# gssales/gaussian-splatting-reflection

Hardware: AMD Instinct MI355X
Metric: train_step_views_per_s (fwd+bwd, 1e6 Gaussians @1080p, surfel rasterizer + reflection path) (higher is better)
Workload: dtype f32

## Files before the change

### gaussian-splatting-reflection_amd/csrc/gsr_common.hip

```cpp
#include "gsr_internal.hpp"
#include <cstdarg>
#include <string>
#include <initializer_list>
#include <vector>
#include <mutex>
#include "gsr_sort.hpp"
#include <rocprim/device/device_scan.hpp>
#include <rocprim/iterator/counting_iterator.hpp>
#include <rocprim/iterator/transform_iterator.hpp>

namespace gsr {

static thread_local char g_err[512] = "";
void set_error(const char* fmt, ...) {
	va_list ap;
	va_start(ap, fmt);
	vsnprintf(g_err, sizeof(g_err), fmt, ap);
	va_end(ap);
}


struct ProfRec {
	int stage;
	hipEvent_t e0, e1;
};
static bool g_prof_on = false;
static std::vector<ProfRec*> g_prof_recs;
static std::vector<ProfRec*> g_prof_free;
static std::mutex g_prof_mu;

StageTimer::StageTimer(int stage_, hipStream_t stream_) : stage(stage_), stream(stream_), rec(nullptr) {
	if (!g_prof_on) return;
	std::lock_guard<std::mutex> lk(g_prof_mu);
	ProfRec* r = nullptr;
	if (!g_prof_free.empty()) {
		r = g_prof_free.back();
		g_prof_free.pop_back();
	} else {
		r = new ProfRec();
		if (hipEventCreate(&r->e0) != hipSuccess || hipEventCreate(&r->e1) != hipSuccess) { delete r; return; }
	}
	r->stage = stage;
	(void)hipEventRecord(r->e0, stream);
	rec = r;
}
StageTimer::~StageTimer() {
	if (!rec) return;
	ProfRec* r = (ProfRec*)rec;
	(void)hipEventRecord(r->e1, stream);
	std::lock_guard<std::mutex> lk(g_prof_mu);
	g_prof_recs.push_back(r);
}

static int g_opt_cull = 1;
int option_cull() { return g_opt_cull; }
static int g_opt_dev = 0;
int option_dev() { return g_opt_dev; }
unsigned long long* dev_pair_counter() {
	static std::mutex mu;
	static unsigned long long* words[64];
	int dev = 0;
	if (hipGetDevice(&dev) != hipSuccess || dev < 0 || dev >= 64) return nullptr;
	std::lock_guard<std::mutex> lk(mu);
	if (!words[dev]) {
		if (hipMalloc((void**)&words[dev], sizeof(unsigned long long)) != hipSuccess) { (void)hipGetLastError(); words[dev] = nullptr; return nullptr; }
		if (hipMemset(words[dev], 0, sizeof(unsigned long long)) != hipSuccess) return nullptr;
	}
	return words[dev];
}
static int g_opt_emit_items = 0;
static int g_opt_mailbox = 1;
static int option_mailbox() { return g_opt_mailbox; }
static int g_opt_sort_driver = GSR_ONESWEEP_DRIVER;
int option_sort_driver() { return GSR_ONESWEEP_DRIVER && g_opt_sort_driver; }

uint32_t higher_msb(uint32_t n) {
	uint32_t msb = sizeof(n) * 4;
	uint32_t step = msb;
	while (step > 1) {
		step /= 2;
		if (n >> msb) msb += step;
		else msb -= step;
	}
	if (n >> msb) msb++;
	return msb;
}

using SortConfig = rocprim::radix_sort_config<rocprim::default_config, rocprim::default_config, rocprim::default_config, 65536>;
#ifndef DEPTH_SORT_BS
#define DEPTH_SORT_BS 1024
#endif
#ifndef DEPTH_SORT_IPT
#define DEPTH_SORT_IPT 4
#endif
#define DEPTH_SORT_SHAPE DEPTH_SORT_BS, DEPTH_SORT_IPT, 8
#define DEPTH_KEY_BITS 31u
#define DEPTH_KEY_PLACES 4u
#ifndef TILE_SORT_IPT
#define TILE_SORT_IPT 16
#endif
#ifndef TILE_SORT_BITS
#define TILE_SORT_BITS 8
#endif
#ifndef TILE_SORT_BS
#define TILE_SORT_BS 1024
#endif
#define TILE_SORT_SHAPE TILE_SORT_BS, TILE_SORT_IPT, TILE_SORT_BITS
#ifndef TILE_SORT_SMALL_FROM
#define TILE_SORT_SMALL_FROM 9000000
#endif
#define TILE_SORT_SHAPE_SMALL TILE_SORT_BS, (TILE_SORT_IPT / 2), TILE_SORT_BITS
#define TILE_SORT_SHAPE_SMALL7 TILE_SORT_BS, (TILE_SORT_IPT / 2), 7
static bool tile_sort_small(size_t R) { return R >= (size_t)TILE_SORT_SMALL_FROM; }
static bool tile_sort_7bit(size_t R, int end_bit) { return tile_sort_small(R) && end_bit > 7 && end_bit <= 14; }
template <class F>
static auto with_tile_sort(size_t R, int end_bit, F&& f) {
	if (tile_sort_7bit(R, end_bit)) return f(RadixSort<TILE_SORT_SHAPE_SMALL7, SortConfig>{});
	if (tile_sort_small(R)) return f(RadixSort<TILE_SORT_SHAPE_SMALL, SortConfig>{});
	return f(RadixSort<TILE_SORT_SHAPE, SortConfig>{});
}
using DepthSort = RadixSort<DEPTH_SORT_SHAPE, SortConfig>;

struct OrderRect {
	const uint32_t* rect;
	int packed;
	__host__ __device__ unsigned long long operator()(uint32_t i) const {
		uint32_t hi = 0u;
		if (packed) {
			const uint2 r = reinterpret_cast<const uint2*>(rect)[i];
			hi = (r.x & 0xFFu) | ((r.x >> 16) << 8) | ((r.y & 0xFFu) << 16) | ((r.y >> 16) << 24);
		}
		return ((unsigned long long)hi << 32) | (unsigned long long)i;
	}
};
using OrderIn = rocprim::transform_iterator<rocprim::counting_iterator<uint32_t>, OrderRect, unsigned long long>;
static OrderIn order_in(const uint32_t* rect, int packed) { return OrderIn(rocprim::counting_iterator<uint32_t>(0), OrderRect{rect, packed}); }

static size_t scan_part_bytes(size_t P) {
	size_t a = 0;
	(void)rocprim::inclusive_scan(nullptr, a, (uint32_t*)nullptr, (uint32_t*)nullptr, P, rocprim::plus<uint32_t>(), 0, false);
	return (a + 255) & ~(size_t)255;
}
size_t sort_temp_bytes(size_t R, int end_bit) {
	return with_tile_sort(R, end_bit, [&](auto sort) { return sort.temp_bytes((uint32_t*)nullptr, (uint32_t*)nullptr, (uint32_t*)nullptr, R, (unsigned)end_bit); });
}

GeomState carve_geom(void* buf, size_t P, const WorkspaceLayout& layout, size_t* total) {
	const size_t scan_bytes = scan_part_bytes(P);
	const size_t sort_bytes = DepthSort::temp_bytes((const uint32_t*)nullptr, order_in(nullptr, 0), (unsigned long long*)nullptr, P, DEPTH_KEY_BITS);
	Carver c(buf);
	GeomState g;
	g.depths = c.take<float>(P);
	g.rect = c.take<uint32_t>(2 * P);
	g.tiles_touched = c.take<uint32_t>(P);
	g.point_offsets = c.take<uint32_t>(P);
	g.clamped = c.take<uint8_t>(P);
	g.rec = c.take<float4>(P * layout.rec_f4);
	g.bbox = c.take<float4>(2 * P);
	g.aux = c.take<float>(P * layout.aux_floats);
	g.acc = c.take<float>(P * layout.acc_floats);
	g.flags = c.take<int>(4);
	g.depth_sorted = c.take<uint32_t>(P);
	g.order = c.take<unsigned long long>(P);
	g.emit_state_bytes = ((((P + 255) / 256 + 1) * sizeof(unsigned long long)) + 15) & ~(size_t)15;
	g.emit_state = c.take<unsigned long long>(g.emit_state_bytes / sizeof(unsigned long long));
	g.scan_temp = c.take<char>(scan_bytes + sort_bytes);
	g.scan_temp_bytes = scan_bytes + sort_bytes;
	g.depth_sort_temp = g.scan_temp ? static_cast<char*>(g.scan_temp) + scan_bytes : nullptr;
	g.depth_sort_bytes = sort_bytes;
	g.depth_sort_clear = DepthSort::cleared_bytes(P, DEPTH_KEY_BITS);
	if (total) *total = c.size();
	return g;
}
ImageState carve_image(void* buf, size_t HW, size_t tiles, const WorkspaceLayout& layout, size_t* total) {
	Carver c(buf);
	ImageState s;
	s.ranges = c.take<uint2>(tiles);
	s.final_T = c.take<float>(HW * layout.planes_T);
	s.n_contrib = c.take<uint32_t>(HW * layout.planes_n);
	s.tile_order = c.take<uint32_t>(tiles);
	if (total) *total = c.size();
	return s;
}
int forward_workspace(gsr_alloc_fn alloc, void* alloc_user, const WorkspaceLayout& layout, size_t P, size_t HW, size_t tiles, GeomState* geom,
                      ImageState* img) {
	size_t geom_bytes = 0, img_bytes = 0;
	carve_geom(nullptr, P, layout, &geom_bytes);
	carve_image(nullptr, HW, tiles, layout, &img_bytes);
	void* gbuf = alloc(alloc_user, GSR_BUF_GEOM, geom_bytes);
	void* ibuf = alloc(alloc_user, GSR_BUF_IMAGE, img_bytes);
	if (!gbuf || !ibuf) { set_error("workspace allocation failed (%zu / %zu bytes)", geom_bytes, img_bytes); return GSR_E_ALLOC; }
	*geom = carve_geom(gbuf, P, layout, nullptr);
	*img = carve_image(ibuf, HW, tiles, layout, nullptr);
	return 0;
}
BinningState carve_binning(void* buf, size_t R, size_t tiles, size_t sort_bytes, size_t* total, bool blend_masks) {
	Carver c(buf);
	BinningState b;
	b.point_list = c.take<uint32_t>(R);
	b.mask_stride = blend_masks ? R / 64 + tiles + 1 : 0;
	b.blend_mask = blend_masks ? c.take<unsigned long long>(16 * b.mask_stride) : nullptr;
	b.tile_keys = c.take<uint32_t>(R);
	b.tile_keys_unsorted = c.take<uint32_t>(R);
	b.vals_unsorted = c.take<uint32_t>(R);
	b.sort_temp = c.take<char>(sort_bytes);
	b.sort_temp_bytes = sort_bytes;
	if (total) *total = c.size();
	return b;
}

#define STATS_BLOCK 1024
__global__ void __launch_bounds__(STATS_BLOCK) gaussian_stats_kernel(int P, const float* __restrict__ depths, const uint32_t* __restrict__ tiles_touched,
                                                                      uint32_t* __restrict__ depth_counts, int* __restrict__ flags, int* __restrict__ mailbox,
                                                                      uint32_t seq) {
	__shared__ uint32_t s_hist[DEPTH_KEY_PLACES * 256u];
	__shared__ unsigned long long s_sum[STATS_BLOCK / 64];
	const uint32_t t = threadIdx.x;
	s_hist[t] = 0u;
	__syncthreads();
	unsigned long long sum = 0ull;
	for (size_t i = (size_t)blockIdx.x * STATS_BLOCK + t; i < (size_t)P; i += (size_t)gridDim.x * STATS_BLOCK) {
		sum += tiles_touched[i];
		if (depth_counts != nullptr) {
			const uint32_t key = __float_as_uint(depths[i]);
			atomicAdd(&s_hist[key & 255u], 1u);
			atomicAdd(&s_hist[256u + ((key >> 8) & 255u)], 1u);
			atomicAdd(&s_hist[512u + ((key >> 16) & 255u)], 1u);
			const uint32_t top = (key >> 24) & 127u;
			unsigned long long todo = __ballot(1);
			while (todo != 0ull) {
				const uint32_t d0 = (uint32_t)__builtin_amdgcn_readlane((int)top, __ffsll((long long)todo) - 1);
				const unsigned long long same = __ballot(top == d0) & todo;
				if ((t & 63u) == (uint32_t)(__ffsll((long long)same) - 1)) atomicAdd(&s_hist[768u + d0], (uint32_t)__popcll(same));
				todo &= ~same;
			}
		}
	}
#pragma unroll
	for (int off = 32; off > 0; off >>= 1) sum += __shfl_xor(sum, off);
	if ((t & 63u) == 0u) s_sum[t >> 6] = sum;
	__syncthreads();
	if (t == 0u) {
		for (uint32_t w = 1; w < STATS_BLOCK / 64; w++) sum += s_sum[w];
		if (sum != 0ull) atomicAdd(reinterpret_cast<unsigned long long*>(flags + 2), sum);
		if (mailbox != nullptr) {
			const uint32_t ticket = __hip_atomic_fetch_add(reinterpret_cast<uint32_t*>(flags + 1), 1u, __ATOMIC_ACQ_REL, __HIP_MEMORY_SCOPE_AGENT);
			if (ticket == gridDim.x - 1u) {
				const unsigned long long total = __hip_atomic_load(reinterpret_cast<unsigned long long*>(flags + 2), __ATOMIC_RELAXED, __HIP_MEMORY_SCOPE_AGENT);
				__hip_atomic_store(mailbox + 2, (int)(uint32_t)(total & 0xFFFFFFFFull), __ATOMIC_RELAXED, __HIP_MEMORY_SCOPE_SYSTEM);
				__hip_atomic_store(mailbox + 3, (int)(uint32_t)(total >> 32), __ATOMIC_RELAXED, __HIP_MEMORY_SCOPE_SYSTEM);
				__hip_atomic_store(reinterpret_cast<uint32_t*>(mailbox + 4), seq, __ATOMIC_RELEASE, __HIP_MEMORY_SCOPE_SYSTEM);
			}
		}
	}
	if (depth_counts != nullptr) {
		const uint32_t h = s_hist[t];
		if (h != 0u) atomicAdd(&depth_counts[t], h);
	}
}
static_assert(STATS_BLOCK == DEPTH_KEY_PLACES * 256u, "one histogram bin per thread");

#ifndef EMIT_BLOCK
#define EMIT_BLOCK 1024
#endif
#define EMIT_BIG 8u
__device__ __forceinline__ unsigned long long emit_pack(uint32_t flag, uint32_t v) { return ((unsigned long long)flag << 62) | (unsigned long long)v; }
__device__ __forceinline__ void emit_publish(unsigned long long* p, unsigned long long v) { __hip_atomic_store(p, v, __ATOMIC_RELAXED, __HIP_MEMORY_SCOPE_AGENT); }
__device__ __forceinline__ unsigned long long emit_peek(unsigned long long* p) { return __hip_atomic_load(p, __ATOMIC_RELAXED, __HIP_MEMORY_SCOPE_AGENT); }

#ifndef EMIT_ITEMS2_FROM
#define EMIT_ITEMS2_FROM 3000000
#endif
template <bool GATHER, int EMIT_ITEMS>
__global__ void __launch_bounds__(EMIT_BLOCK) emit_tiles_kernel(int P, const unsigned long long* __restrict__ order, const uint32_t* __restrict__ rect,
                                                         unsigned long long* __restrict__ scan_state, uint32_t* __restrict__ ticket,
                                                         uint32_t* __restrict__ tile_keys, uint32_t* __restrict__ vals, uint32_t tiles_x,
                                                         uint2* __restrict__ ranges, uint32_t tiles, void* sort_clear, size_t sort_clear_bytes,
                                                         unsigned long long* __restrict__ blend_mask, size_t blend_words) {
	__shared__ uint32_t s_wsum[EMIT_BLOCK / 64];
	__shared__ uint32_t s_base;
	__shared__ uint32_t s_bid;
	if (threadIdx.x == 0) s_bid = __hip_atomic_fetch_add(ticket, 1u, __ATOMIC_RELAXED, __HIP_MEMORY_SCOPE_AGENT);
	__syncthreads();
	const int bid = (int)s_bid;
	const size_t gtid = (size_t)bid * EMIT_BLOCK + threadIdx.x;
	const uint32_t lane = threadIdx.x & 63u, wave = threadIdx.x >> 6;
	const int i0 = (bid * EMIT_BLOCK + (int)threadIdx.x) * EMIT_ITEMS;
	uint32_t idx[EMIT_ITEMS], x0[EMIT_ITEMS], y0[EMIT_ITEMS], x1[EMIT_ITEMS], y1[EMIT_ITEMS], cnt[EMIT_ITEMS];
	unsigned long long ov[EMIT_ITEMS];
	if (EMIT_ITEMS == 2 && i0 + 1 < P) {
		const ulonglong2 o2 = *reinterpret_cast<const ulonglong2*>(order + i0);
		ov[0] = o2.x; ov[EMIT_ITEMS - 1] = o2.y;
	} else {
#pragma unroll
		for (int e = 0; e < EMIT_ITEMS; e++) ov[e] = i0 + e < P ? order[i0 + e] : 0ull;
	}
	uint32_t mine = 0u;
#pragma unroll
	for (int e = 0; e < EMIT_ITEMS; e++) {
		idx[e] = (uint32_t)ov[e];
		x0[e] = y0[e] = x1[e] = y1[e] = 0u;
		if (i0 + e < P) {
			if (GATHER) {
				const uint2 r = reinterpret_cast<const uint2*>(rect)[idx[e]];
				x0[e] = r.x & 0xFFFFu; y0[e] = r.x >> 16; x1[e] = r.y & 0xFFFFu; y1[e] = r.y >> 16;
			} else {
				const uint32_t hi = (uint32_t)(ov[e] >> 32);
				x0[e] = hi & 0xFFu; y0[e] = (hi >> 8) & 0xFFu; x1[e] = (hi >> 16) & 0xFFu; y1[e] = hi >> 24;
			}
		}
		cnt[e] = (x1[e] - x0[e]) * (y1[e] - y0[e]);
		mine += cnt[e];
	}
	for (size_t t = gtid; t < blend_words; t += (size_t)gridDim.x * EMIT_BLOCK) blend_mask[t] = 0ull;
	for (uint32_t t = (uint32_t)gtid; t < tiles; t += gridDim.x * EMIT_BLOCK) ranges[t] = make_uint2(0u, 0u);
	sort_clear_region(sort_clear, sort_clear_bytes, gtid, (size_t)gridDim.x * EMIT_BLOCK);
	uint32_t incl = mine;
#pragma unroll
	for (uint32_t o = 1; o < 64; o <<= 1) {
		const uint32_t v = __shfl_up(incl, o, 64);
		if (lane >= o) incl += v;
	}
	if (lane == 63u) s_wsum[wave] = incl;
	__syncthreads();
	if (wave == 0u) {
		uint32_t total = 0u;
		for (uint32_t w = 0; w < EMIT_BLOCK / 64; w++) total += s_wsum[w];
		uint32_t prefix = 0u;
		if (bid == 0) {
			if (lane == 0u) emit_publish(scan_state, emit_pack(2u, total));
		} else {
			if (lane == 0u) emit_publish(scan_state + bid, emit_pack(1u, total));
			int j = bid - 1;
			for (;;) {
				const int tgt = j - (int)lane;
				const unsigned long long st = tgt >= 0 ? emit_peek(scan_state + tgt) : emit_pack(2u, 0u);
				const uint32_t flag = (uint32_t)(st >> 62);
				const unsigned long long done = __ballot(flag == 2u), empty = __ballot(flag == 0u);
				const int stop = done != 0ull ? __ffsll((long long)done) - 1 : 63;
				const unsigned long long need = stop == 63 ? ~0ull : ((2ull << stop) - 1ull);
				if ((empty & need) != 0ull) continue;
				uint32_t v = (int)lane <= stop ? (uint32_t)st : 0u;
#pragma unroll
				for (int o = 32; o > 0; o >>= 1) v += __shfl_xor(v, o);
				prefix += v;
				if (done != 0ull) break;
				j -= 64;
			}
			if (lane == 0u) emit_publish(scan_state + bid, emit_pack(2u, prefix + total));
		}
		if (lane == 0u) s_base = prefix;
	}
	__syncthreads();
	uint32_t wbase = s_base;
	for (uint32_t w = 0; w < wave; w++) wbase += s_wsum[w];
	uint32_t off = wbase + incl - mine;
#pragma unroll
	for (int e = 0; e < EMIT_ITEMS; e++) {
		if (cnt[e] != 0u && cnt[e] <= EMIT_BIG) {
			uint32_t o = off;
			for (uint32_t y = y0[e]; y < y1[e]; y++)
				for (uint32_t x = x0[e]; x < x1[e]; x++) {
					tile_keys[o] = y * tiles_x + x;
					vals[o] = idx[e];
					o++;
				}
		}
		unsigned long long big = __ballot(cnt[e] > EMIT_BIG);
		while (big) {
			const int src = __ffsll((long long)big) - 1;
			big &= big - 1;
			const uint32_t b_off = (uint32_t)__builtin_amdgcn_readlane((int)off, src), b_cnt = (uint32_t)__builtin_amdgcn_readlane((int)cnt[e], src);
			const uint32_t b_idx = (uint32_t)__builtin_amdgcn_readlane((int)idx[e], src);
			const uint32_t b_x0 = (uint32_t)__builtin_amdgcn_readlane((int)x0[e], src), b_y0 = (uint32_t)__builtin_amdgcn_readlane((int)y0[e], src);
			const uint32_t b_w = (uint32_t)__builtin_amdgcn_readlane((int)(x1[e] - x0[e]), src);
			for (uint32_t q = lane; q < b_cnt; q += 64u) {
				const uint32_t dy = q / b_w, dx = q - dy * b_w;
				tile_keys[b_off + q] = (b_y0 + dy) * tiles_x + (b_x0 + dx);
				vals[b_off + q] = b_idx;
			}
		}
		off += cnt[e];
	}
}

__global__ void __launch_bounds__(256) tile_ranges_kernel(int L, const uint32_t* __restrict__ tile_keys, uint2* __restrict__ ranges) {
	const int idx = blockIdx.x * 256 + threadIdx.x;
	if (idx >= L) return;
	const uint32_t currtile = tile_keys[idx];
	if (idx == 0) ranges[currtile].x = 0;
	else {
		const uint32_t prevtile = tile_keys[idx - 1];
		if (currtile != prevtile) {
			ranges[prevtile].y = idx;
			ranges[currtile].x = idx;
		}
	}
	if (idx == L - 1) ranges[currtile].y = L;
}

#define TILE_ORDER_REGS 16
__global__ void __launch_bounds__(1024) tile_order_kernel(int tiles, const uint2* __restrict__ ranges, uint32_t* __restrict__ order) {
	__shared__ uint32_t hist[1024];
	__shared__ uint32_t s_wave[16];
	__shared__ uint32_t s_max;
	const int t = threadIdx.x;
	hist[t] = 0;
	if (t == 0) s_max = 0;
	uint32_t len[TILE_ORDER_REGS];
	uint32_t m = 0;
#pragma unroll
	for (int j = 0; j < TILE_ORDER_REGS; j++) {
		const int i = t + 1024 * j;
		const uint2 r = i < tiles ? ranges[i] : make_uint2(0u, 0u);
		len[j] = r.y - r.x;
		m = max(m, len[j]);
	}
	for (int i = t + 1024 * TILE_ORDER_REGS; i < tiles; i += 1024) m = max(m, ranges[i].y - ranges[i].x);
	__syncthreads();
	atomicMax(&s_max, m);
	__syncthreads();
	int shift = 0;
	while ((s_max >> shift) >= 1024u) shift++;
#pragma unroll
	for (int j = 0; j < TILE_ORDER_REGS; j++)
		if (t + 1024 * j < tiles) atomicAdd(&hist[1023u - (len[j] >> shift)], 1u);
	for (int i = t + 1024 * TILE_ORDER_REGS; i < tiles; i += 1024) atomicAdd(&hist[1023u - ((ranges[i].y - ranges[i].x) >> shift)], 1u);
	__syncthreads();
	const uint32_t mine = hist[t];
	uint32_t incl = mine;
	const int lane = t & 63, wave = t >> 6;
#pragma unroll
	for (int off = 1; off < 64; off <<= 1) {
		const uint32_t o = __shfl_up(incl, off, 64);
// ... 47 lines not shown
			unsigned spins = 0;
			while (box[4] != seq) {
				if ((++spins & 63u) == 0u && hipStreamQuery(stream) != hipErrorNotReady) break;
			}
			if (box[4] != seq) {
				GSR_HIP_CHECK(hipStreamSynchronize(stream));
				if (box[4] != seq) { set_error("num_rendered mailbox was not written"); return GSR_E_HIP; }
			}
			__atomic_thread_fence(__ATOMIC_ACQUIRE);
		} else {
			GSR_HIP_CHECK(hipEventSynchronize(done));
		}
		memcpy(total, word + 2, sizeof(*total));
		*trap = word[0];
		return 0;
	}
};
static Readback* readback_slot() {
	static thread_local Readback slots[64];
	int dev = 0;
	if (hipGetDevice(&dev) != hipSuccess || dev < 0 || dev >= 64) return nullptr;
	Readback& r = slots[dev];
	if (!r.word) {
		if (hipHostMalloc((void**)&r.word, 64, hipHostMallocMapped | hipHostMallocCoherent) == hipSuccess) {
			if (hipHostGetDevicePointer((void**)&r.dev_word, r.word, 0) != hipSuccess) r.dev_word = nullptr;
		} else {
			(void)hipGetLastError();
			r.dev_word = nullptr;
			if (hipHostMalloc((void**)&r.word, 64, hipHostMallocDefault) != hipSuccess) { r.word = nullptr; return nullptr; }
		}
		memset(r.word, 0, 64);
	}
	if (!r.done && hipEventCreateWithFlags(&r.done, hipEventDisableTiming) != hipSuccess) { r.done = nullptr; return nullptr; }
	return &r;
}

static int rect_packs(int tiles_x, int tiles_y) { return (tiles_x <= 255 && tiles_y <= 255) ? 1 : 0; }

int run_binning(gsr_alloc_fn alloc, void* alloc_user, int P, int tiles_x, int tiles_y, const GeomState& geom, const ImageState& img,
                BinningState* out_binning, int prefiltered, int debug, hipStream_t stream, bool blend_masks) {
	Readback* rb = readback_slot();
	if (!rb) { set_error("pinned word / event for the num_rendered readback could not be created"); return GSR_E_HIP; }
	{
		StageTimer st_(GSR_STAGE_SCAN, stream);
		const unsigned blocks = (unsigned)std::min<size_t>(512, ((size_t)P + 4 * STATS_BLOCK - 1) / (4 * STATS_BLOCK));
		int* mailbox = rb->begin(prefiltered);
		gaussian_stats_kernel<<<blocks, STATS_BLOCK, 0, stream>>>(P, geom.depths, geom.tiles_touched,
		                                                          geom.depth_sort_clear ? reinterpret_cast<uint32_t*>(geom.depth_sort_temp) : nullptr, geom.flags, mailbox,
		                                                          rb->seq);
		GSR_LAUNCH_CHECK(debug, stream);
		const int rc = rb->copy_back(geom.flags, stream);
		if (rc < 0) return rc;
	}
	{
		StageTimer st_(GSR_STAGE_SORT, stream);
		GSR_HIP_CHECK(DepthSort::pairs(geom.depth_sort_temp, geom.depth_sort_bytes, reinterpret_cast<const uint32_t*>(geom.depths), geom.depth_sorted,
		                               order_in(geom.rect, rect_packs(tiles_x, tiles_y)), geom.order, (size_t)P, DEPTH_KEY_BITS, stream, true,
		                               reinterpret_cast<const uint32_t*>(geom.depth_sort_temp)));
	}
	unsigned long long total64;
	int trap;
	const int waited = rb->wait(stream, &total64, &trap);
	if (waited < 0) return waited;
	if (prefiltered && trap != 0) { set_error("Point is filtered although prefiltered is set. This shouldn't happen!"); return GSR_E_PREFILTERED; }
	if (total64 > 0x7fffffffull) { set_error("num_rendered = %llu does not fit the int the API returns", total64); return GSR_E_INVALID; }
	const int R = (int)total64;
	const uint32_t tiles = (uint32_t)tiles_x * (uint32_t)tiles_y;
	const int bit = (int)higher_msb(tiles);
	const size_t sort_bytes = R > 0 ? sort_temp_bytes((size_t)R, bit) : 0;
	size_t total = 0;
	carve_binning(nullptr, (size_t)R, (size_t)tiles, sort_bytes, &total, blend_masks);
	void* buf = alloc(alloc_user, GSR_BUF_BINNING, total);
	if (!buf && total > 0) { set_error("binning buffer allocation of %zu bytes failed", total); return GSR_E_ALLOC; }
	BinningState b = carve_binning(buf, (size_t)R, (size_t)tiles, sort_bytes, nullptr, blend_masks);
	*out_binning = b;

	if (R == 0) GSR_HIP_CHECK(hipMemsetAsync(img.ranges, 0, (size_t)tiles * sizeof(uint2), stream));
	if (R > 0) {
		{
			StageTimer st_(GSR_STAGE_EMIT_KEYS, stream);
			const size_t clear_bytes = with_tile_sort((size_t)R, bit, [&](auto sort) { return sort.cleared_bytes((size_t)R, (unsigned)bit); });
			uint32_t* ticket = reinterpret_cast<uint32_t*>(geom.emit_state + (geom.emit_state_bytes / sizeof(unsigned long long) - 1));
			const int items = g_opt_emit_items ? g_opt_emit_items : (P >= EMIT_ITEMS2_FROM ? 2 : 1);
			auto emit = rect_packs(tiles_x, tiles_y) ? (items == 2 ? emit_tiles_kernel<false, 2> : emit_tiles_kernel<false, 1>)
			                                         : (items == 2 ? emit_tiles_kernel<true, 2> : emit_tiles_kernel<true, 1>);
			emit<<<(P + EMIT_BLOCK * items - 1) / (EMIT_BLOCK * items), EMIT_BLOCK, 0, stream>>>(P, geom.order, geom.rect, geom.emit_state, ticket, b.tile_keys_unsorted,
			                                                       b.vals_unsorted, (uint32_t)tiles_x, img.ranges, tiles, b.sort_temp, clear_bytes, b.blend_mask,
			                                                       16 * b.mask_stride);
		}
		GSR_LAUNCH_CHECK(debug, stream);
		{
			StageTimer st_(GSR_STAGE_SORT, stream);
			GSR_HIP_CHECK(with_tile_sort((size_t)R, bit, [&](auto sort) {
				return sort.pairs(b.sort_temp, b.sort_temp_bytes, b.tile_keys_unsorted, b.tile_keys, b.vals_unsorted, b.point_list, (size_t)R, (unsigned)bit, stream, true);
			}));
		}
		if (debug) GSR_HIP_CHECK(hipStreamSynchronize(stream));
		{
			StageTimer st_(GSR_STAGE_RANGES, stream);
			tile_ranges_kernel<<<(R + 255) / 256, 256, 0, stream>>>(R, b.tile_keys, img.ranges);
		}
		GSR_LAUNCH_CHECK(debug, stream);
	}
	{
		StageTimer st_(GSR_STAGE_RANGES, stream);
		const int rc = run_tile_order(img, tiles, stream);
		if (rc < 0) return rc;
	}
	return R;
}

int run_tile_order(const ImageState& img, size_t tiles, hipStream_t stream) {
	if (tiles == 0) return 0;
	tile_order_kernel<<<1, 1024, 0, stream>>>((int)tiles, img.ranges, img.tile_order);
	GSR_LAUNCH_CHECK(0, stream);
	return 0;
}

__global__ void __launch_bounds__(256) mark_visible_kernel(int P, const float* __restrict__ pts, const float* __restrict__ vm,
                                                           uint8_t* __restrict__ present) {
#pragma clang fp contract(off)
	const int idx = blockIdx.x * 256 + threadIdx.x;
	if (idx >= P) return;
	const float x = pts[3 * idx], y = pts[3 * idx + 1], z = pts[3 * idx + 2];
	const float pz = vm[2] * x + vm[6] * y + vm[10] * z + vm[14];
	present[idx] = (pz <= 0.2f) ? 0 : 1;
}

__global__ void __launch_bounds__(256) widen_clamped_kernel(int P, const uint8_t* __restrict__ packed, uint8_t* __restrict__ out) {
	const int idx = blockIdx.x * 256 + threadIdx.x;
	if (idx >= P) return;
	const uint8_t b = packed[idx];
	out[3 * idx + 0] = b & 1;
	out[3 * idx + 1] = (b >> 1) & 1;
	out[3 * idx + 2] = (b >> 2) & 1;
}
struct RecPick { int n; int pos[9]; };
__global__ void __launch_bounds__(256) pick_rec_kernel(int P, const float* __restrict__ rec, int stride, RecPick pick, float* __restrict__ out) {
	const int i = blockIdx.x * 256 + threadIdx.x;
	if (i >= P * pick.n) return;
	const int idx = i / pick.n, k = i % pick.n;
	out[i] = rec[(size_t)idx * stride + pick.pos[k]];
}
__global__ void __launch_bounds__(256) gather_rec_kernel(int P, const float* __restrict__ rec, int stride, int first, int nf,
                                                         float* __restrict__ out) {
	const int i = blockIdx.x * 256 + threadIdx.x;
	if (i >= P * nf) return;
	const int idx = i / nf, k = i % nf;
	out[i] = rec[(size_t)idx * stride + first + k];
}

}

using namespace gsr;

extern "C" const char* gsr_last_error(void) { return g_err; }
extern "C" int gsr_version(void) { return GSR_ABI_VERSION; }


extern "C" int gsr_set_option(const char* name, int value) {
	if (std::string(name) == "cull") { g_opt_cull = value ? 1 : 0; return 0; }
	if (std::string(name) == "dev") { g_opt_dev = value; return 0; }
	if (std::string(name) == "emit_items") { g_opt_emit_items = (value == 1 || value == 2) ? value : 0; return 0; }
	if (std::string(name) == "mailbox") { g_opt_mailbox = value ? 1 : 0; return 0; }
	if (std::string(name) == "sort_driver") { g_opt_sort_driver = value ? 1 : 0; return 0; }
	set_error("gsr_set_option: unknown option '%s'", name);
	return GSR_E_INVALID;
}
extern "C" int gsr_profile_enable(int on) {
	std::lock_guard<std::mutex> lk(g_prof_mu);
	for (ProfRec* r : g_prof_recs) g_prof_free.push_back(r);
	g_prof_recs.clear();
	g_prof_on = on != 0;
	return 0;
}
extern "C" int gsr_profile_collect(float* ms_out, int* launches_out) {
	std::lock_guard<std::mutex> lk(g_prof_mu);
	for (int i = 0; i < GSR_STAGE_COUNT; i++) { if (ms_out) ms_out[i] = 0.f; if (launches_out) launches_out[i] = 0; }
	for (ProfRec* r : g_prof_recs) {
		float ms = 0.f;
		if (hipEventSynchronize(r->e1) == hipSuccess && hipEventElapsedTime(&ms, r->e0, r->e1) == hipSuccess) {
			if (ms_out) ms_out[r->stage] += ms;
			if (launches_out) launches_out[r->stage] += 1;
		}
		g_prof_free.push_back(r);
	}
	g_prof_recs.clear();
	return 0;
}

extern "C" int gsr_mark_visible(int P, const float* means3D, const float* viewmatrix, const float* projmatrix, uint8_t* present,
                                void* stream_) {
	(void)projmatrix;
	hipStream_t stream = (hipStream_t)stream_;
	if (P < 0 || (P > 0 && (!means3D || !viewmatrix || !present))) { set_error("gsr_mark_visible: invalid argument"); return GSR_E_INVALID; }
	if (P == 0) return 0;
	mark_visible_kernel<<<(P + 255) / 256, 256, 0, stream>>>(P, means3D, viewmatrix, present);
	GSR_LAUNCH_CHECK(0, stream);
	return 0;
}

extern "C" int gsr_debug_fetch(int variant, const char* name, int P, int R, int width, int height, const void* geom_buffer,
                               const void* binning_buffer, const void* image_buffer, void* dst, void* stream_) {
	hipStream_t stream = (hipStream_t)stream_;
	const int tiles_x = (width + 15) / 16, tiles_y = (height + 15) / 16;
	const size_t HW = (size_t)width * height, tiles = (size_t)tiles_x * tiles_y;
	const WorkspaceLayout& layout = variant == 0 ? SURFEL_LAYOUT : GAUSS_LAYOUT;
	const int stride = layout.rec_f4 * 4;
	GeomState g = carve_geom((void*)geom_buffer, P, layout, nullptr);
	ImageState im = carve_image((void*)image_buffer, HW, tiles, layout, nullptr);
	BinningState b = carve_binning((void*)binning_buffer, R, tiles, 0, nullptr);
	auto d2d = [&](const void* src, size_t bytes) -> int {
		if (bytes == 0) return 0;
		GSR_HIP_CHECK(hipMemcpyAsync(dst, src, bytes, hipMemcpyDeviceToDevice, stream));
		return 0;
	};
	auto gather = [&](int first, int nf) -> int {
		if (P == 0) return 0;
		gather_rec_kernel<<<(P * nf + 255) / 256, 256, 0, stream>>>(P, (const float*)g.rec, stride, first, nf, (float*)dst);
		GSR_LAUNCH_CHECK(0, stream);
		return 0;
	};
	std::string n(name);
	if (n == "pairs") {
		const unsigned long long* word = dev_pair_counter();
		if (!word) { set_error("gsr_debug_fetch: no pair counter"); return GSR_E_HIP; }
		return d2d(word, sizeof(unsigned long long));
	}
	if (n == "depths") return d2d(g.depths, (size_t)P * 4);
	if (n == "means2D") return gather(0, 2);

	if (n == "tiles_touched") return d2d(g.tiles_touched, (size_t)P * 4);
	if (n == "cull") return d2d(g.bbox, (size_t)P * 32);
	if (n == "point_offsets") {
		if (P == 0) return 0;
		size_t tmp = (size_t)(static_cast<char*>(g.depth_sort_temp) - static_cast<char*>(g.scan_temp));
		GSR_HIP_CHECK(rocprim::inclusive_scan(g.scan_temp, tmp, g.tiles_touched, g.point_offsets, (size_t)P, rocprim::plus<uint32_t>(), stream, false));
		return d2d(g.point_offsets, (size_t)P * 4);
	}
	if (n == "clamped") {
		if (P == 0) return 0;
		widen_clamped_kernel<<<(P + 255) / 256, 256, 0, stream>>>(P, g.clamped, (uint8_t*)dst);
		GSR_LAUNCH_CHECK(0, stream);
		return 0;
	}
	auto pick = [&](std::initializer_list<int> pos) -> int {
		if (P == 0) return 0;
		RecPick pk;
		pk.n = (int)pos.size();
		int i = 0;
		for (int v : pos) pk.pos[i++] = v;
		pick_rec_kernel<<<(P * pk.n + 255) / 256, 256, 0, stream>>>(P, (const float*)g.rec, stride, pk, (float*)dst);
		GSR_LAUNCH_CHECK(0, stream);
		return 0;
	};
	if (n == "rgb") return variant == 0 ? gather(16, 3) : gather(6, 3);
	if (n == "geom4") {
		return variant == 0 ? pick({12, 13, 14, 11}) : gather(2, 4);
	}
	if (n == "transMat" && variant == 0) return pick({2, 4, 6, 3, 5, 7, 8, 9, 10});
	if (n == "cov3D" && variant == 1) { set_error("gsr_debug_fetch: the 3D covariance is not kept by the forward (round 4: the backward recomputes it)"); return GSR_E_INVALID; }
	if (n == "point_list") return d2d(b.point_list, (size_t)R * 4);
	if (n == "blend_mask") return d2d(b.blend_mask, 16 * b.mask_stride * sizeof(unsigned long long));
	if (n == "keys") {
		if (R == 0) return 0;
		rebuild_keys_kernel<<<(R + 255) / 256, 256, 0, stream>>>(R, b.tile_keys, b.point_list, g.depths, (uint64_t*)dst);
		GSR_LAUNCH_CHECK(0, stream);
		return 0;
	}
	if (n == "ranges") return d2d(im.ranges, tiles * 8);
	if (n == "final_T") return d2d(im.final_T, HW * 4 * layout.planes_T);
	if (n == "n_contrib") return d2d(im.n_contrib, HW * 4 * layout.planes_n);
	set_error("gsr_debug_fetch: unknown array '%s'", name);
	return GSR_E_INVALID;
}
```

### gaussian-splatting-reflection_amd/csrc/gsr_cubemap.hip

```cpp
#include <algorithm>
#include <cstring>
#include "gsr_internal.hpp"
#include <mutex>
#include <memory>
#include "gsr_sort.hpp"
#include <rocprim/iterator/counting_iterator.hpp>
#include "gsr_refl.hpp"

namespace gsr {



struct Plain {
	int f, ux0, ux1, uy0, uy1;
	float kx, ky;
};
__device__ __forceinline__ void plain_index(float vx, float vy, float vz, int L, Plain& p, bool nearest) {
	float u, v;
	cube_uv(vx, vy, vz, u, v, p.f);
	v = -v;
	u = (u * 0.5f + 0.5f) * (float)L;
	v = (v * 0.5f + 0.5f) * (float)L;
	if (nearest) {
		p.ux0 = min(max((int)u, 0), L - 1);
// ... 239 lines not shown
			lg1 *= 0.5f * (float)L * graw;
			if (s.flag & 1) lg0 = -lg0;
			if (s.flag & 4) lg1 = -lg1;
			lg1 = -lg1;
			cube_uv_backward(face, o.rx, o.ry, o.rz, lg0, lg1, grx, gry, grz);
		}
	}
	{
		const bool inA = ((threadIdx.x >> 2) & 1) == 0;
		const int XOR4 = 0x101F;
		const int s_i0 = inA ? tix[1] : tix[0], s_i1 = inA ? tix[3] : tix[2];
		const float s_w0 = inA ? twg[1] : twg[0], s_w1 = inA ? twg[3] : twg[2];
		const int r_i0 = __builtin_amdgcn_ds_swizzle(s_i0, XOR4), r_i1 = __builtin_amdgcn_ds_swizzle(s_i1, XOR4);
		const float r_w0 = __int_as_float(__builtin_amdgcn_ds_swizzle(__float_as_int(s_w0), XOR4));
		const float r_w1 = __int_as_float(__builtin_amdgcn_ds_swizzle(__float_as_int(s_w1), XOR4));
		const int i0 = inA ? tix[0] : r_i0, i1 = inA ? tix[2] : r_i1, i2 = inA ? r_i0 : tix[1], i3 = inA ? r_i1 : tix[3];
		const float w0 = inA ? twg[0] : r_w0, w1 = inA ? twg[2] : r_w1, w2 = inA ? r_w0 : twg[1], w3 = inA ? r_w1 : twg[3];
		if (i0 >= 0) atomicAdd(g_scratch + i0, w0);
		if (i1 >= 0) atomicAdd(g_scratch + i1, w1);
		if (i2 >= 0) atomicAdd(g_scratch + i2, w2);
		if (i3 >= 0) atomicAdd(g_scratch + i3, w3);
	}
	gs = quad_sum(gs); grx = quad_sum(grx); gry = quad_sum(gry); grz = quad_sum(grz);
	if (live && ch == 3) g_strength[p] = gs;
	const float grn = grx * o.nx + gry * o.ny + grz * o.nz;
	float gnx = -2.f * (o.dn * grx + grn * o.dx);
	float gny = -2.f * (o.dn * gry + grn * o.dy);
	float gnz = -2.f * (o.dn * grz + grn * o.dz);
	if (g_nworld) { gnx += g_nworld[p]; gny += g_nworld[HW + p]; gnz += g_nworld[2 * HW + p]; }
	const float inv = refl_rcp(o.len + 1e-6f);
	float gwx = gnx * inv, gwy = gny * inv, gwz = gnz * inv;
	if (o.len > 0.f) {
		const float k = (o.nwx * gnx + o.nwy * gny + o.nwz * gnz) * inv * inv * refl_rcp(o.len);
		gwx -= o.nwx * k; gwy -= o.nwy * k; gwz -= o.nwz * k;
	}
	if (chan) g_normal_view[c * HW + p] = gwx * cam[c] + gwy * cam[3 + c] + gwz * cam[6 + c];
}

#ifndef ENTRIES_BS
#define ENTRIES_BS 512
#endif
template <bool RGBA>
__global__ void __launch_bounds__(ENTRIES_BS)
deferred_refl_bwd_entries_kernel(const float* __restrict__ normal_view, const float* __restrict__ base, const float* __restrict__ strength,
                                 const float* __restrict__ cam, const float* __restrict__ cubemap, const float4* __restrict__ rgba,
                                 const float* __restrict__ fail_value, int L,
                                 int W, int H, const float* __restrict__ g_final, const float* __restrict__ g_refl_color,
                                 const float* __restrict__ g_nworld, float* __restrict__ g_normal_view, float* __restrict__ g_base,
                                 float* __restrict__ g_strength, float* __restrict__ g_fail, float* __restrict__ g_scratch,
                                 ReflFootprint* __restrict__ footprints, uint32_t* __restrict__ keys, const uint32_t* __restrict__ keys_fwd, uint32_t no_key,
                                 void* sort_clear, size_t sort_clear_bytes) {
	const size_t HW = (size_t)W * H;
	const size_t pix = (size_t)blockIdx.x * ENTRIES_BS + threadIdx.x;
	sort_clear_region(sort_clear, sort_clear_bytes, pix, (size_t)gridDim.x * ENTRIES_BS);
	const bool live = pix < HW;
	const size_t p = live ? pix : 0;
	const int py = (int)(p / W), px = (int)(p - (size_t)py * W);
	ReflBwdIn in;
	in.nvx = normal_view[p]; in.nvy = normal_view[HW + p]; in.nvz = normal_view[2 * HW + p];
	in.sv = strength[p];
	in.has_grc = g_refl_color != nullptr;
	in.has_gnw = g_nworld != nullptr;
#pragma unroll
	for (int c = 0; c < 3; c++) {
		in.gfin[c] = g_final[c * HW + p];
		in.bas[c] = base[c * HW + p];
		in.grc[c] = g_refl_color ? g_refl_color[c * HW + p] : 0.f;
		in.gnw[c] = g_nworld ? g_nworld[c * HW + p] : 0.f;
	}
	const uint32_t kf = keys_fwd ? keys_fwd[p] : no_key;
	ReflBwdOut o;
	refl_backward_pixel<RGBA>(cam, cubemap, rgba, fail_value, L, px, py, live, in, g_fail, g_scratch, footprints + p, keys_fwd != nullptr, kf,
	                          keys ? keys + p : nullptr, no_key, (int)(threadIdx.x & 63), o);
	if (!live) return;
	g_strength[p] = o.g_strength;
#pragma unroll
	for (int c = 0; c < 3; c++) {
		g_base[c * HW + p] = o.g_base[c];
		g_normal_view[c * HW + p] = o.g_nv[c];
	}
}

template <bool ACC>
__global__ void __launch_bounds__(256) unpack_cubemap_grad_kernel(const float4* __restrict__ scratch, float* __restrict__ g_cubemap,
                                                                  float* __restrict__ g_fail, int L) {
	const size_t n = (size_t)6 * L * L;
	const size_t t = (size_t)blockIdx.x * 256 + threadIdx.x;
	if (t == 0) {
		const float4 gf = scratch[n];
		g_fail[0] = (ACC ? g_fail[0] : 0.f) + gf.x; g_fail[1] = (ACC ? g_fail[1] : 0.f) + gf.y; g_fail[2] = (ACC ? g_fail[2] : 0.f) + gf.z;
	}
	if (t >= n) return;
	const size_t LL = (size_t)L * L;
	const size_t f = t / LL, r = t - f * LL;
	const float4 g = scratch[t];
	float* o = g_cubemap + f * 3 * LL + r;
	o[0] = (ACC ? o[0] : 0.f) + g.x;
	o[LL] = (ACC ? o[LL] : 0.f) + g.y;
	o[2 * LL] = (ACC ? o[2 * LL] : 0.f) + g.z;
}

#define REFL_CHUNK 8
#ifndef REFL_WIN
#define REFL_WIN 1024u
#endif
__global__ void __launch_bounds__(256) refl_run_combine_kernel(const uint32_t* __restrict__ keys_sorted, const uint32_t* __restrict__ pix_sorted,
                                                               const ReflFootprint* __restrict__ footprints, size_t n, uint32_t L, uint32_t no_key,
                                                               float* __restrict__ g_scratch) {
	__shared__ float win[3][REFL_WIN];
	__shared__ uint32_t s_hi;
	const size_t wg0 = (size_t)blockIdx.x * 256 * REFL_CHUNK;
	const uint32_t t_lo = keys_sorted[wg0];
	if (t_lo == no_key) return;
	const size_t wg_last = min(n, wg0 + (size_t)256 * REFL_CHUNK) - 1;
	const uint32_t t_hi = keys_sorted[wg_last];
	const uint32_t reach = t_hi == no_key ? REFL_WIN : min(REFL_WIN, t_hi - t_lo + L + 2u);
	for (uint32_t i = threadIdx.x; i < reach; i += 256) { win[0][i] = 0.f; win[1][i] = 0.f; win[2][i] = 0.f; }
	if (threadIdx.x == 0) s_hi = 0u;
	__syncthreads();

	const size_t i0 = wg0 + (size_t)threadIdx.x * REFL_CHUNK;
	uint32_t key[REFL_CHUNK];
	float4 ga[REFL_CHUNK];
	float gky[REFL_CHUNK];
#pragma unroll
	for (int j = 0; j < REFL_CHUNK; j++) key[j] = i0 + j < n ? keys_sorted[i0 + j] : no_key;
#pragma unroll
	for (int j = 0; j < REFL_CHUNK; j++) {
		ga[j] = make_float4(0.f, 0.f, 0.f, 0.f);
		gky[j] = 0.f;
		if (key[j] != no_key) {
			const float* f = reinterpret_cast<const float*>(footprints + pix_sorted[i0 + j]);
			ga[j] = *reinterpret_cast<const float4*>(f);
			gky[j] = f[4];
		}
	}
	float acc[4][3];
	uint32_t cur = no_key, hi = 0u;
	auto flush = [&]() {
		if (cur == no_key) return;
#pragma unroll
		for (int k = 0; k < 4; k++) {
			const uint32_t rel = cur - t_lo + (uint32_t)(k & 1) + (uint32_t)(k >> 1) * L;
			if (rel < REFL_WIN) {
				hi = max(hi, rel);
#pragma unroll
				for (int c = 0; c < 3; c++)
					if (acc[k][c] != 0.f) atomicAdd(&win[c][rel], acc[k][c]);
			} else {
				float* dst = g_scratch + (((size_t)t_lo + rel) << 2);
#pragma unroll
				for (int c = 0; c < 3; c++)
					if (acc[k][c] != 0.f) atomicAdd(dst + c, acc[k][c]);
			}
		}
	};
#pragma unroll
	for (int j = 0; j < REFL_CHUNK; j++) {
		if (key[j] != no_key) {
			if (key[j] != cur) {
				flush();
				cur = key[j];
#pragma unroll
				for (int k = 0; k < 4; k++) { acc[k][0] = 0.f; acc[k][1] = 0.f; acc[k][2] = 0.f; }
			}
			const float kx = ga[j].w, ky = gky[j];
			const float w4[4] = {(1 - ky) * (1 - kx), (1 - ky) * kx, ky * (1 - kx), ky * kx};
#pragma unroll
			for (int k = 0; k < 4; k++) {
				acc[k][0] += w4[k] * ga[j].x; acc[k][1] += w4[k] * ga[j].y; acc[k][2] += w4[k] * ga[j].z;
			}
		}
	}
	flush();
	if (hi != 0u) atomicMax(&s_hi, hi);
	__syncthreads();
	const uint32_t top = s_hi;
	for (uint32_t i = threadIdx.x; i <= top; i += 256) {
// ... 120 lines not shown
};
std::mutex g_side_mu;
SideStream g_side[64];
SideStream* side_stream(bool create) {
	int dev = 0;
	if (hipGetDevice(&dev) != hipSuccess || dev < 0 || dev >= 64) return nullptr;
	SideStream& s = g_side[dev];
	if (!s.stream && create) {
		int least = 0, greatest = 0;
		(void)hipDeviceGetStreamPriorityRange(&least, &greatest);
		if (hipStreamCreateWithPriority(&s.stream, hipStreamNonBlocking, greatest) != hipSuccess) { s.stream = nullptr; return nullptr; }
		if (hipEventCreateWithFlags(&s.fork, hipEventDisableTiming) != hipSuccess || hipEventCreateWithFlags(&s.fork2, hipEventDisableTiming) != hipSuccess ||
		    hipEventCreateWithFlags(&s.done, hipEventDisableTiming) != hipSuccess || hipEventCreateWithFlags(&s.gate, hipEventDisableTiming) != hipSuccess) {
			(void)hipStreamDestroy(s.stream);
			s.stream = nullptr;
		}
	}
	return s.stream ? &s : nullptr;
}

struct ReflTail {
	ReflScratch rs;
	float* staging = nullptr;
	float* fail_acc = nullptr;
	ReflFootprint* footprints = nullptr;
	uint32_t *keys_in = nullptr, *keys_out = nullptr, *pix_out = nullptr;
	void* sort_temp = nullptr;
	hipStream_t stream, tail;
	SideStream* side = nullptr;
	std::unique_lock<std::mutex> lock;

	ReflTail(uint32_t L, int width, int height, hipStream_t s) : rs(refl_scratch(L, width, height)), stream(s), tail(s) {}
	bool carve(float* scratch, size_t scratch_floats) {
		staging = scratch;
		fail_acc = scratch + rs.ntex * 4;
		if (scratch_floats < rs.total_floats || rs.n >= ((size_t)1 << 30) || rs.ntex >= 0xFFFFFFFFull || ((uintptr_t)scratch & 31) != 0) return false;
		footprints = reinterpret_cast<ReflFootprint*>(scratch + (rs.ntex + 1) * 4 + 4);
		keys_in = reinterpret_cast<uint32_t*>(footprints + rs.n);
		keys_out = keys_in + rs.n;
		pix_out = keys_out + rs.n;
		sort_temp = reinterpret_cast<void*>(((uintptr_t)(pix_out + rs.n) + 255) & ~(uintptr_t)255);
		return true;
	}
	void lock_side() { lock = std::unique_lock<std::mutex>(g_side_mu); }
	void use_side_stream() {
		lock_side();
		side = side_stream(true);
		if (side) tail = side->stream;
	}
	size_t sort_cleared_bytes(bool small) const {
		return with_refl_sort(rs.key_bits, small, [&](auto sort) { return sort.cleared_bytes(rs.n, (unsigned)rs.key_bits); });
	}
	hipError_t fork(hipEvent_t ev) {
		hipError_t e = hipEventRecord(ev, stream);
		return e == hipSuccess ? hipStreamWaitEvent(side->stream, ev, 0) : e;
	}
	hipError_t sort(const uint32_t* keys, bool small, bool gated) {
		hipError_t e = with_refl_sort(rs.key_bits, small, [&](auto sort) {
			return sort.pairs(sort_temp, rs.sort_bytes, keys, keys_out, rocprim::counting_iterator<uint32_t>(0), pix_out, rs.n, (unsigned)rs.key_bits, tail, true, nullptr,
			                  gated && side ? side->gate : nullptr);
		});
		if (e == hipSuccess && gated && side) side->gate_pending = true;
		return e;
	}
	hipError_t mark_done() {
		hipError_t e = hipEventRecord(side->done, side->stream);
		if (e == hipSuccess) side->recorded = true;
		return e;
	}
};
}

namespace gsr {
int side_gate_wait(hipStream_t stream) {
	std::lock_guard<std::mutex> lk(g_side_mu);
	SideStream* s = side_stream(false);
	if (s && s->gate_pending) {
		s->gate_pending = false;
		GSR_HIP_CHECK(hipStreamWaitEvent(stream, s->gate, 0));
	}
	return 0;
}

int refl_sort_keys_early(uint32_t L, int width, int height, float* scratch, size_t scratch_floats, const uint32_t* sort_keys, int async, bool gated,
                         hipStream_t stream) {
	ReflTail t(L, width, height, stream);
	if (!t.carve(scratch, scratch_floats)) {
		set_error("reflection backward (sorted footprints): scratch of %zu floats, 32-byte aligned, needed (gsr_deferred_reflection_scratch_floats(L, W, H, 1))",
		          t.rs.total_floats);
		return GSR_E_INVALID;
	}
	if (async) t.use_side_stream();
	if (t.side) GSR_HIP_CHECK(t.fork(t.side->fork));
	{
		StageTimer tt(GSR_STAGE_REFL_BWD_TAIL, t.tail);
		GSR_HIP_CHECK(hipMemsetAsync(t.sort_temp, 0, t.sort_cleared_bytes(false), t.tail));
		GSR_HIP_CHECK(t.sort(sort_keys, false, gated));
	}
	if (t.side) GSR_HIP_CHECK(t.mark_done());
	return 0;
}
}

extern "C" int gsr_side_join(void* stream_) {
	std::lock_guard<std::mutex> lk(g_side_mu);
	const SideStream* s = side_stream(false);
	if (s && s->recorded) GSR_HIP_CHECK(hipStreamWaitEvent((hipStream_t)stream_, s->done, 0));
	return 0;
}

extern "C" int gsr_deferred_reflection_backward_keys(const float* normal_view, const float* base_color, const float* refl_strength, const float* cam,
                                                   const float* cubemap, const float* fail_value, uint32_t L, int width, int height,
                                                   const float* g_final, const float* g_refl_color, const float* g_normal_world,
                                                   float* g_normal_view, float* g_base, float* g_strength, float* g_cubemap, float* g_fail,
                                                   float* scratch, size_t scratch_floats, int accumulate, int async_tail, const float* cubemap_rgba,
                                                   const uint32_t* sort_keys, int keys_sorted, void* stream_) {
	hipStream_t stream = (hipStream_t)stream_;
	if (width <= 0 || height <= 0 || !normal_view || !base_color || !refl_strength || !cam || !cubemap || !fail_value || !g_final ||
	    !g_normal_view || !g_base || !g_strength || !g_cubemap || !g_fail || !scratch || L == 0 || (keys_sorted && !sort_keys)) {
		set_error("gsr_deferred_reflection_backward: invalid argument");
		return GSR_E_INVALID;
	}
	const size_t HW = (size_t)width * height;
	ReflTail t(L, width, height, stream);
	const size_t ntex = t.rs.ntex;
	if (scratch_floats < (ntex + 1) * 4) { set_error("gsr_deferred_reflection_backward: scratch smaller than (6*L*L+1)*4 floats"); return GSR_E_INVALID; }
	const bool binned = t.carve(scratch, scratch_floats);
	if (keys_sorted && !binned) { set_error("gsr_deferred_reflection_backward: keys_sorted needs the scratch the forward sorted into"); return GSR_E_INVALID; }
	auto unpack = accumulate ? unpack_cubemap_grad_kernel<true> : unpack_cubemap_grad_kernel<false>;
	GSR_HIP_CHECK(hipMemsetAsync(scratch, 0, (ntex + 1) * 4 * sizeof(float), stream));
	if (!binned) {
		{
			StageTimer st_(GSR_STAGE_REFL_BWD, stream);
			const unsigned grid = (unsigned)((HW * 4 + 255) / 256);
			deferred_refl_bwd_kernel<<<grid, 256, 0, stream>>>(normal_view, base_color, refl_strength, cam, cubemap, fail_value, (int)L, width, height, g_final,
			                                                  g_refl_color, g_normal_world, g_normal_view, g_base, g_strength, t.staging, t.fail_acc);
		}
		unpack<<<(unsigned)((ntex + 255) / 256), 256, 0, stream>>>((const float4*)t.staging, g_cubemap, g_fail, (int)L);
		GSR_LAUNCH_CHECK(0, stream);
		return 0;
	}
	const bool small_sort = async_tail && !sort_keys;
	const size_t sort_cleared = t.sort_cleared_bytes(small_sort);
	if (async_tail) t.use_side_stream();
	else if (keys_sorted) t.lock_side();
	if (keys_sorted) {
		const SideStream* s = side_stream(false);
		if (s && s->recorded && t.tail != s->stream) GSR_HIP_CHECK(hipStreamWaitEvent(t.tail, s->done, 0));
	} else if (sort_keys) {
		GSR_HIP_CHECK(hipMemsetAsync(t.sort_temp, 0, sort_cleared, stream));
		if (t.side) GSR_HIP_CHECK(t.fork(t.side->fork));
		StageTimer tt(GSR_STAGE_REFL_BWD_TAIL, t.tail);
		GSR_HIP_CHECK(t.sort(sort_keys, false, true));
	}
	{
		StageTimer st_(GSR_STAGE_REFL_BWD, stream);
		const unsigned egrid = (unsigned)((HW + ENTRIES_BS - 1) / ENTRIES_BS);
		if (cubemap_rgba && ((uintptr_t)cubemap_rgba & 15) == 0)
			deferred_refl_bwd_entries_kernel<true><<<egrid, ENTRIES_BS, 0, stream>>>(normal_view, base_color, refl_strength, cam, cubemap,
			                                                                 reinterpret_cast<const float4*>(cubemap_rgba), fail_value, (int)L, width, height, g_final,
			                                                                 g_refl_color, g_normal_world, g_normal_view, g_base, g_strength, t.fail_acc, t.staging,
			                                                                 t.footprints, t.keys_in, sort_keys, (uint32_t)ntex, sort_keys ? nullptr : t.sort_temp,
			                                                                 sort_keys ? 0 : sort_cleared);
		else
			deferred_refl_bwd_entries_kernel<false><<<egrid, ENTRIES_BS, 0, stream>>>(normal_view, base_color, refl_strength, cam, cubemap, nullptr, fail_value, (int)L, width,
			                                                                  height, g_final, g_refl_color, g_normal_world, g_normal_view, g_base, g_strength, t.fail_acc,
			                                                                  t.staging, t.footprints, t.keys_in, sort_keys, (uint32_t)ntex, sort_keys ? nullptr : t.sort_temp,
			                                                                  sort_keys ? 0 : sort_cleared);
	}
	if (t.side) GSR_HIP_CHECK(t.fork(sort_keys ? t.side->fork2 : t.side->fork));
	{
		StageTimer tt(GSR_STAGE_REFL_BWD_TAIL, t.tail);
		const size_t per_wg = (size_t)256 * REFL_CHUNK;
		const unsigned cgrid = (unsigned)((t.rs.n + per_wg - 1) / per_wg);
		if (!sort_keys) GSR_HIP_CHECK(t.sort(t.keys_in, small_sort, false));
		refl_run_combine_kernel<<<cgrid, 256, 0, t.tail>>>(t.keys_out, t.pix_out, t.footprints, t.rs.n, L, (uint32_t)ntex, t.staging);
		unpack<<<(unsigned)((ntex + 255) / 256), 256, 0, t.tail>>>((const float4*)t.staging, g_cubemap, g_fail, (int)L);
	}
	if (t.side) GSR_HIP_CHECK(t.mark_done());
	GSR_HIP_CHECK(hipGetLastError());
	return 0;
}

extern "C" int gsr_deferred_reflection_backward_ex(const float* normal_view, const float* base_color, const float* refl_strength, const float* cam,
                                                   const float* cubemap, const float* fail_value, uint32_t L, int width, int height,
                                                   const float* g_final, const float* g_refl_color, const float* g_normal_world,
                                                   float* g_normal_view, float* g_base, float* g_strength, float* g_cubemap, float* g_fail,
                                                   float* scratch, size_t scratch_floats, int accumulate, int async_tail, const float* cubemap_rgba,
                                                   void* stream_) {
	return gsr_deferred_reflection_backward_keys(normal_view, base_color, refl_strength, cam, cubemap, fail_value, L, width, height, g_final, g_refl_color,
	                                             g_normal_world, g_normal_view, g_base, g_strength, g_cubemap, g_fail, scratch, scratch_floats, accumulate,
	                                             async_tail, cubemap_rgba, nullptr, 0, stream_);
}

extern "C" int gsr_deferred_reflection_backward_accum(const float* normal_view, const float* base_color, const float* refl_strength, const float* cam,
                                                const float* cubemap, const float* fail_value, uint32_t L, int width, int height,
                                                const float* g_final, const float* g_refl_color, const float* g_normal_world,
                                                float* g_normal_view, float* g_base, float* g_strength, float* g_cubemap, float* g_fail,
                                                float* scratch, size_t scratch_floats, int accumulate, void* stream_) {
	return gsr_deferred_reflection_backward_keys(normal_view, base_color, refl_strength, cam, cubemap, fail_value, L, width, height, g_final, g_refl_color,
	                                             g_normal_world, g_normal_view, g_base, g_strength, g_cubemap, g_fail, scratch, scratch_floats, accumulate, 0, nullptr,
	                                             nullptr, 0, stream_);
}

extern "C" int gsr_deferred_reflection_backward(const float* normal_view, const float* base_color, const float* refl_strength, const float* cam,
                                                const float* cubemap, const float* fail_value, uint32_t L, int width, int height,
                                                const float* g_final, const float* g_refl_color, const float* g_normal_world,
                                                float* g_normal_view, float* g_base, float* g_strength, float* g_cubemap, float* g_fail,
                                                float* scratch, size_t scratch_floats, void* stream_) {
	return gsr_deferred_reflection_backward_accum(normal_view, base_color, refl_strength, cam, cubemap, fail_value, L, width, height, g_final, g_refl_color,
	                                              g_normal_world, g_normal_view, g_base, g_strength, g_cubemap, g_fail, scratch, scratch_floats, 0, stream_);
}

__global__ void __launch_bounds__(256) normal_world_fwd_kernel(const float* __restrict__ normal_view, const float* __restrict__ cam, size_t HW,
                                                               float* __restrict__ out) {
	const size_t pix = (size_t)blockIdx.x * 256 + threadIdx.x;
	if (pix >= HW) return;
	const float vx = normal_view[pix], vy = normal_view[HW + pix], vz = normal_view[2 * HW + pix];
	const float wx = vx * cam[0] + vy * cam[1] + vz * cam[2], wy = vx * cam[3] + vy * cam[4] + vz * cam[5], wz = vx * cam[6] + vy * cam[7] + vz * cam[8];
	const float inv = 1.0f / (sqrtf(wx * wx + wy * wy + wz * wz) + 1e-6f);
	out[pix] = wx * inv; out[HW + pix] = wy * inv; out[2 * HW + pix] = wz * inv;
}
__global__ void __launch_bounds__(256) normal_world_bwd_kernel(const float* __restrict__ normal_view, const float* __restrict__ cam, size_t HW,
                                                               const float* __restrict__ g_out, float* __restrict__ g_normal_view) {
	const size_t pix = (size_t)blockIdx.x * 256 + threadIdx.x;
	if (pix >= HW) return;
	const float vx = normal_view[pix], vy = normal_view[HW + pix], vz = normal_view[2 * HW + pix];
	const float wx = vx * cam[0] + vy * cam[1] + vz * cam[2], wy = vx * cam[3] + vy * cam[4] + vz * cam[5], wz = vx * cam[6] + vy * cam[7] + vz * cam[8];
	const float len = sqrtf(wx * wx + wy * wy + wz * wz);
	const float inv = 1.0f / (len + 1e-6f);
	const float gx = g_out[pix], gy = g_out[HW + pix], gz = g_out[2 * HW + pix];
	float ax = gx * inv, ay = gy * inv, az = gz * inv;
	if (len > 0.f) {
		const float k = (wx * gx + wy * gy + wz * gz) * inv * inv / len;
		ax -= wx * k; ay -= wy * k; az -= wz * k;
	}
#pragma unroll
	for (int c = 0; c < 3; c++) g_normal_view[c * HW + pix] = ax * cam[c] + ay * cam[3 + c] + az * cam[6 + c];
}
extern "C" int gsr_normal_world_forward(const float* normal_view, const float* cam, int width, int height, float* out_normal_world, void* stream_) {
	if (width <= 0 || height <= 0 || !normal_view || !cam || !out_normal_world) { set_error("gsr_normal_world_forward: invalid argument"); return GSR_E_INVALID; }
	const size_t HW = (size_t)width * height;
	normal_world_fwd_kernel<<<(unsigned)((HW + 255) / 256), 256, 0, (hipStream_t)stream_>>>(normal_view, cam, HW, out_normal_world);
	GSR_LAUNCH_CHECK(0, (hipStream_t)stream_);
	return 0;
}
extern "C" int gsr_normal_world_backward(const float* normal_view, const float* cam, int width, int height, const float* g_normal_world,
                                         float* g_normal_view, void* stream_) {
	if (width <= 0 || height <= 0 || !normal_view || !cam || !g_normal_world || !g_normal_view) { set_error("gsr_normal_world_backward: invalid argument"); return GSR_E_INVALID; }
	const size_t HW = (size_t)width * height;
	normal_world_bwd_kernel<<<(unsigned)((HW + 255) / 256), 256, 0, (hipStream_t)stream_>>>(normal_view, cam, HW, g_normal_world, g_normal_view);
	GSR_LAUNCH_CHECK(0, (hipStream_t)stream_);
	return 0;
}
```

### gaussian-splatting-reflection_amd/csrc/gsr_gauss.hip

```cpp
#include "gsr_internal.hpp"
#include "gsr_tile_walk.hpp"
#include "gsr_sort.hpp"
#include "gsr_math.hpp"

namespace gsr {

#define GA_COLOR 0
#define GA_NORMAL 3
#define GA_REFL 6
#define GA_INVD 7
#define GA_MEAN2D 8
#define GA_MEAN2DP 10
#define GA_CONIC 12
#define GA_OPAC 15

__device__ __forceinline__ void cov3d_from_scale_rot(const float* __restrict__ scale, float mod, const float* __restrict__ rot, float* cov3D) {
#pragma clang fp contract(off)
	M3 S = m3_make(1, 0, 0, 0, 1, 0, 0, 0, 1);
	S.m[0][0] = mod * scale[0];
	S.m[1][1] = mod * scale[1];
	S.m[2][2] = mod * scale[2];
	const float r = rot[0], x = rot[1], y = rot[2], z = rot[3];
	M3 R = m3_make(1.f - 2.f * (y * y + z * z), 2.f * (x * y - r * z), 2.f * (x * z + r * y), 2.f * (x * y + r * z),
	               1.f - 2.f * (x * x + z * z), 2.f * (y * z - r * x), 2.f * (x * z - r * y), 2.f * (y * z + r * x),
// ... 47 lines not shown
		if (prefiltered) g.flags[0] = 1;
		return false;
	}
	const float hx = pm[0] * mx + pm[4] * my + pm[8] * mz + pm[12];
	const float hy = pm[1] * mx + pm[5] * my + pm[9] * mz + pm[13];
	const float hw = pm[3] * mx + pm[7] * my + pm[11] * mz + pm[15];
	const float p_w = 1.0f / (hw + 0.0000001f);
	const float projx = hx * p_w, projy = hy * p_w;

	if (cov3D_precomp != nullptr) {
#pragma unroll
		for (int i = 0; i < 6; i++) cov3D[i] = cov3D_precomp[6 * idx + i];
	} else {
		cov3d_from_scale_rot(scales + 3 * idx, scale_modifier, rotations + 4 * idx, cov3D);
	}
	const Cov2DCtx k = cov2d_ctx(mx, my, mz, cam);
	const M3 Vrk = m3_make(cov3D[0], cov3D[1], cov3D[2], cov3D[1], cov3D[3], cov3D[4], cov3D[2], cov3D[4], cov3D[5]);
	const M3 cov = m3_mul(m3_mul(m3_T(k.T), m3_T(Vrk)), k.T);
	float cx = cov.m[0][0], cy = cov.m[0][1], cz = cov.m[1][1];
	const float h_var = 0.3f;
	const float det_cov = cx * cz - cy * cy;
	cx += h_var;
	cz += h_var;
	const float det = cx * cz - cy * cy;
	float h_convolution_scaling = 1.0f;
	if (antialiasing) h_convolution_scaling = sqrtf(fmaxf(0.000025f, det_cov / det));
	if (det == 0.0f) return false;
	const float det_inv = 1.f / det;
	const float conx = cz * det_inv, cony = -cy * det_inv, conz = cx * det_inv;
	const float mid = 0.5f * (cx + cz);
	const float lambda1 = mid + sqrtf(fmaxf(0.1f, mid * mid - det));
	const float lambda2 = mid - sqrtf(fmaxf(0.1f, mid * mid - det));
	const float my_radius = ceilf(3.f * sqrtf(fmaxf(lambda1, lambda2)));
	const float pix_x = (float)((((double)projx + 1.0) * cam.W - 1.0) * 0.5);
	const float pix_y = (float)((((double)projy + 1.0) * cam.H - 1.0) * 0.5);
	uint32_t x0, y0, x1, y1;
	get_rect(pix_x, pix_y, f2i(my_radius), gx, gy, x0, y0, x1, y1);
	if ((x1 - x0) * (y1 - y0) == 0) return false;

	float cr, cg, cb;
	if (colors_precomp == nullptr) {
		const float dx = mx - cam.campos[0], dy = my - cam.campos[1], dz = mz - cam.campos[2];
		const float len = sqrtf(dx * dx + dy * dy + dz * dz);
		ShRow s;
		load_sh(shs, idx, M, (D + 1) * (D + 1), s);
		const F3 c = sh_eval(D, s, dx / len, dy / len, dz / len);
		g.clamped[idx] = (uint8_t)((c.x < 0 ? 1 : 0) | (c.y < 0 ? 2 : 0) | (c.z < 0 ? 4 : 0));
		cr = fmaxf(c.x, 0.0f); cg = fmaxf(c.y, 0.0f); cb = fmaxf(c.z, 0.0f);
	} else {
		cr = colors_precomp[3 * idx]; cg = colors_precomp[3 * idx + 1]; cb = colors_precomp[3 * idx + 2];
	}
	g.depths[idx] = pvz;
	radii[idx] = f2i(my_radius);
	g.rect[2 * idx] = x0 | (y0 << 16);
	g.rect[2 * idx + 1] = x1 | (y1 << 16);
	float4* rec = o;
	rec[0] = make_float4(pix_x, pix_y, conx, cony);
	rec[1] = make_float4(conz, opacities[idx] * h_convolution_scaling, cr, cg);
	rec[2] = make_float4(cb, normals[3 * idx], normals[3 * idx + 1], normals[3 * idx + 2]);
	rec[3] = make_float4(refl[idx], 1.0f / pvz, 0.f, 0.f);
	{
		const float opac = opacities[idx] * h_convolution_scaling;
		float4 c0 = make_float4(pix_x, pix_y, 0.f, 0.f), c1 = make_float4(0.f, 0.f, 0.f, -2.0f);
		if (opac >= 1.0f / 255.0f) {
			const float inv_q = 1.0f / (2.0f * logf(255.0f * opac) * 1.05f + 0.1f);
			c0.z = conx * inv_q; c0.w = cony * inv_q; c1.x = conz * inv_q; c1.w = -1.0f;
		}
		o[G_REC_F4] = c0;
		o[G_REC_F4 + 1] = c1;
	}
	g.tiles_touched[idx] = (y1 - y0) * (x1 - x0);
	return true;
}

__global__ void __launch_bounds__(256)
gauss_preprocess_kernel(int P, int D, int M, const float* __restrict__ means, const float* __restrict__ scales, float scale_modifier,
                        const float* __restrict__ rotations, const float* __restrict__ opacities, const float* __restrict__ shs,
                        const float* __restrict__ cov3D_precomp, const float* __restrict__ colors_precomp, const float* __restrict__ normals,
                        const float* __restrict__ refl, RasterCam cam, int* __restrict__ radii, GeomState g, int gx, int gy, int prefiltered,
                        int antialiasing) {
	const int idx = blockIdx.x * 256 + threadIdx.x;
	sort_clear_region(g.depth_sort_temp, g.depth_sort_clear, (size_t)idx, (size_t)gridDim.x * 256u);
	sort_clear_region(g.emit_state, g.emit_state_bytes, (size_t)idx, (size_t)gridDim.x * 256u);
	if (idx == 0) { g.flags[1] = 0; g.flags[2] = 0; g.flags[3] = 0; }
	__shared__ float4 s_out[4][6 * 65];
	const int lane = threadIdx.x & 63;
	float4* so = s_out[threadIdx.x >> 6];
	float4 o[G_REC_F4 + 2];
	float cov3D[6] = {0.f, 0.f, 0.f, 0.f, 0.f, 0.f};
#pragma unroll
	for (int k = 0; k < G_REC_F4 + 2; k++) o[k] = make_float4(0.f, 0.f, 0.f, 0.f);
	bool live = false;
	if (idx < P)
		live = gauss_preprocess_one(idx, D, M, means, scales, scale_modifier, rotations, opacities, shs, cov3D_precomp, colors_precomp, normals, refl, cam,
		                            radii, g, gx, gy, prefiltered, antialiasing, o, cov3D);
	if (__ballot(live) == 0ull) return;
	const int g0 = idx - lane;
	const int ng = min(64, P - g0);
	wave_store_rows4<G_REC_F4, false>(so, o, g.rec + (size_t)g0 * G_REC_F4, G_REC_F4, 0, ng, lane);
	wave_store_rows4<2, false>(so, o + G_REC_F4, g.bbox + (size_t)g0 * 2, 2, 0, ng, lane);
}

__device__ __forceinline__ lmask gauss_pair(float4 r0, float conz, float opac, float pixx, float pixy, float& dx, float& dy, float& G,
                                            float& alpha) {
#pragma clang fp contract(off)
	dx = r0.x - pixx;
	dy = r0.y - pixy;
	const float q = fmaf(r0.z * dx, dx, (conz * dy) * dy);
	const float power = fmaf(-0.5f, q, -((r0.w * dx) * dy));
	G = __expf(power);
	alpha = fminf(0.99f, opac * G);
	return LMASK(!(power > 0.0f)) & LMASK(!(alpha < 1.0f / 255.0f));
}

#define G_SUB 16
template <bool INVDEPTH, bool COUNT = false>
__global__ void __launch_bounds__(64)
gauss_render_fwd_wave_kernel(const uint2* __restrict__ ranges, const uint32_t* __restrict__ tile_order, const uint32_t* __restrict__ point_list, int W, int H, int tiles_x, int ntiles,
                             const float4* __restrict__ rec, const float4* __restrict__ bbox, int cull, const float* __restrict__ bg,
                             float* __restrict__ final_T, uint32_t* __restrict__ n_contrib, float* __restrict__ out_color,
                             float* __restrict__ out_normal, float* __restrict__ out_refl, float* __restrict__ out_invdepth,
                             unsigned long long* __restrict__ blend_mask, size_t mask_stride, PairCount<COUNT> pairs) {
	const uint32_t slot = xcd_slot(blockIdx.x);
	if (slot >= (uint32_t)ntiles * 4u) return;
	const TileBlock blk = tile_block(tile_order, slot, tiles_x);
	if (blk.bx0 >= W || blk.by0 >= H) return;
	const uint32_t tile = blk.tile, quad = blk.quad;
	const int lane = threadIdx.x, bx0 = blk.bx0, by0 = blk.by0;
	const int px = bx0 + (lane & 7), py = by0 + (lane >> 3);
	const bool inside = px < W && py < H;
	const float pixx = (float)px, pixy = (float)py;
	const uint2 range = ranges[tile];
	const int count = (int)(range.y - range.x);
	const float qx0 = (float)bx0, qy0 = (float)by0;

	__shared__ uint32_t s_hid[WBATCH];
	__shared__ uint32_t s_hj[WBATCH];

	lmask done = ~LMASK(px < W) | ~LMASK(py < H);
	LiveBox<false> box(qx0, qy0);
	uint32_t npairs = 0;
	float T = 1.0f;
	uint32_t last_contributor = 0;
	float C0 = 0, C1 = 0, C2 = 0, N0 = 0, N1 = 0, N2 = 0, RS = 0, ID = 0;
	const size_t batch0 = (size_t)(range.x / WBATCH) + tile;

	for (int base = 0; base < count; base += WBATCH) {
		if (done == ~0ull) break;
		const int nb = min(WBATCH, count - base);
		bool hit = lane < nb;
		uint32_t id = 0;
		if (!pairs.whole_block()) box.refresh(done, qx0, qy0);
		if (hit) {
			id = point_list[range.x + (uint32_t)(base + lane)];
			if (cull) {
				hit = cull_hit(bbox[2 * id], bbox[2 * id + 1], box.x0, box.x1, box.y0, box.y1);
			}
		}
		const unsigned long long mm = __ballot(hit);
		const int nh = __popcll(mm);
		if (nh == 0) continue;
		const HitList hl = compact_hits(hit, mm, nh, lane, id, (uint32_t)lane, s_hid, s_hj);
		const int kown = hl.kown;
		const uint32_t hid = hl.a, hj = hl.b;
		__syncthreads();
		unsigned long long blendk = 0ull;
		using Rec = TileRec<G_REC_F4>;
		auto fetch = [&](int k) { return fetch_rec<G_REC_F4>(rec, hid, k); };
		auto blend = [&](int k, const Rec& R, auto&& prefetch_next) -> bool {
			const uint32_t contributor = (uint32_t)(base + (int)__builtin_amdgcn_readlane(hj, k) + 1);
			if constexpr (COUNT) npairs++;
			float dx, dy, G, alpha;
			const lmask live = gauss_pair(R.f[0], R.f[1].x, R.f[1].y, pixx, pixy, dx, dy, G, alpha) & ~done;
			__builtin_amdgcn_sched_barrier(0);
			prefetch_next();
			__builtin_amdgcn_sched_barrier(0);
			const float test_T = T * (1 - alpha);
			const lmask sat = LMASK(test_T < 0.0001f) & live;
			const lmask ok = live & ~sat;
			done |= sat;
			if (ok != 0ull) {
				const float w = selm0(ok, alpha * T);
				C0 = fmaf(R.f[1].z, w, C0); C1 = fmaf(R.f[1].w, w, C1); C2 = fmaf(R.f[2].x, w, C2);
				N0 = fmaf(R.f[2].y, w, N0); N1 = fmaf(R.f[2].z, w, N1); N2 = fmaf(R.f[2].w, w, N2);
				RS = fmaf(R.f[3].x, w, RS);
				if (INVDEPTH) ID = fmaf(R.f[3].y, w, ID);
				T = selm(ok, test_T, T);
				last_contributor = selmu(ok, contributor, last_contributor);
				blendk |= 1ull << k;
			}
			return done == ~0ull;
		};
		Rec A = fetch(0), B = A;
		for (int k = 0; k < nh; k += 2) {
			if (blend(k, A, [&]() { if (k + 1 < nh) B = fetch(k + 1); })) break;
			if (k + 1 >= nh) break;
			if (blend(k + 1, B, [&]() { if (k + 2 < nh) A = fetch(k + 2); })) break;
		}
		const lmask blended = __ballot(hit && ((blendk >> kown) & 1ull) != 0ull);
		if (lane == 0) blend_mask[(size_t)quad * mask_stride + batch0 + (size_t)(base / WBATCH)] = blended;
	}
	if constexpr (COUNT) {
		if (lane == 0) atomicAdd(pairs.word, (unsigned long long)npairs);
	}
	if (inside) {
		const size_t HW = (size_t)H * W;
		const size_t pix = (size_t)W * py + px;
		final_T[pix] = T;
		n_contrib[pix] = last_contributor;
		out_color[pix] = C0 + T * bg[0];
		out_color[HW + pix] = C1 + T * bg[1];
		out_color[2 * HW + pix] = C2 + T * bg[2];
		out_normal[pix] = N0;
		out_normal[HW + pix] = N1;
		out_normal[2 * HW + pix] = N2;
		out_refl[pix] = RS;
		if (INVDEPTH) out_invdepth[pix] = ID;
	}
}

template <bool INVDEPTH>
__global__ void __launch_bounds__(64)
gauss_render_bwd_wave_kernel(const uint2* __restrict__ ranges, const uint32_t* __restrict__ tile_order, const uint32_t* __restrict__ point_list, int W, int H, int tiles_x, int ntiles,
                             const float* __restrict__ bg, const float4* __restrict__ rec, const float4* __restrict__ bbox, int cull,
                             const float* __restrict__ final_Ts, const uint32_t* __restrict__ n_contrib, const float* __restrict__ dL_dpixels,
                             const float* __restrict__ dL_dnormal_map, const float* __restrict__ dL_drefl_map,
                             const float* __restrict__ dL_invdepths, float* __restrict__ acc, const unsigned long long* __restrict__ blend_mask,
                             size_t mask_stride) {
	const uint32_t slot = xcd_slot(blockIdx.x);
	if (slot >= (uint32_t)ntiles * 4u) return;
	const TileBlock blk = tile_block(tile_order, slot, tiles_x);
	if (blk.bx0 >= W || blk.by0 >= H) return;
	const uint32_t tile = blk.tile, quad = blk.quad;
	const int lane = threadIdx.x, bx0 = blk.bx0, by0 = blk.by0;
	const int px = bx0 + (lane & 7), py = by0 + (lane >> 3);
	const bool inside = px < W && py < H;
	const float pixx = (float)px, pixy = (float)py;
	const uint2 range = ranges[tile];
	const int count = (int)(range.y - range.x);
	const size_t HW = (size_t)H * W;
	const size_t pix = (size_t)W * py + px;
	__shared__ float s_slab[G_SUB * 4 * G_ACC_F];
	__shared__ uint32_t s_hid[WBATCH];
	__shared__ uint32_t s_hj[WBATCH];

	const lmask inside_m = LMASK(px < W) & LMASK(py < H);
	const uint32_t slab_lane = (uint32_t)(lane >> 4) * G_ACC_F + (uint32_t)row_reduce_slot(lane);
	const float T_final = inside ? final_Ts[pix] : 0.f;
	float T = T_final;
	const int last_contributor = inside ? (int)n_contrib[pix] : 0;
	float dp0 = 0, dp1 = 0, dp2 = 0, dn0 = 0, dn1 = 0, dn2 = 0, dr = 0, di = 0;
	if (inside) {
		dp0 = dL_dpixels[pix]; dp1 = dL_dpixels[HW + pix]; dp2 = dL_dpixels[2 * HW + pix];
		dn0 = dL_dnormal_map[pix]; dn1 = dL_dnormal_map[HW + pix]; dn2 = dL_dnormal_map[2 * HW + pix];
		dr = dL_drefl_map[pix];
		if (INVDEPTH) di = dL_invdepths[pix];
	}
	float A1 = 0, A2 = 0, D1p = 0, D2p = 0, last_alpha = 0;
	const float dp0x3 = 3.0f * dp0, dp1x2 = 2.0f * dp1;
	const float ddelx_dx = 0.5f * W, ddely_dy = 0.5f * H;
	const float bg_dot_dpixel = bg[0] * dp0 + bg[1] * dp1 + bg[2] * dp2;

	int wave_last = last_contributor;
#pragma unroll
	for (int off = 32; off > 0; off >>= 1) wave_last = max(wave_last, __shfl_xor(wave_last, off));
	wave_last = __builtin_amdgcn_readfirstlane(wave_last);
	if (wave_last == 0) return;
	const size_t batch0 = (size_t)(range.x / WBATCH) + tile;
	for (int b = (min(wave_last, count) - 1) / WBATCH; b >= 0; b--) {
		const unsigned long long bits = blend_mask[(size_t)quad * mask_stride + batch0 + (size_t)b];
		if (bits == 0ull) continue;
		const int pos = b * WBATCH + (WBATCH - 1 - lane);
		const bool hit = ((bits >> (WBATCH - 1 - lane)) & 1ull) != 0ull && pos < wave_last;
		const unsigned long long mm = __ballot(hit);
		const int nh = __popcll(mm);
		if (nh == 0) continue;
		const HitList hl = compact_hits(hit, mm, nh, lane, hit ? point_list[range.x + (uint32_t)pos] : 0u, (uint32_t)pos, s_hid, s_hj);
		const uint32_t hid = hl.a, hj = hl.b;
		unsigned long long touched = 0ull;
		using Rec = TileRec<G_REC_F4>;
		auto fetch = [&](int k) { return fetch_rec<G_REC_F4>(rec, hid, k); };
		auto differentiate = [&](int k, const Rec& R, auto&& prefetch_next) {
			const int contributor = (int)__builtin_amdgcn_readlane(hj, k);
			float dx, dy, Gp, alpha_p;
			const lmask ok = gauss_pair(R.f[0], R.f[1].x, R.f[1].y, pixx, pixy, dx, dy, Gp, alpha_p) & LMASK(contributor < last_contributor) & inside_m;
			__builtin_amdgcn_sched_barrier(0);
			prefetch_next();
			__builtin_amdgcn_sched_barrier(0);
			if (ok == 0ull) return;
			float v[G_ACC_F];
			const float alpha = selm0(ok, alpha_p), G = selm0(ok, Gp);
			const float inv_1ma = div_nr(1.0f, 1.f - alpha);
			T *= inv_1ma;
			const float w = alpha * T;
			float D1 = R.f[1].z * dp0 + R.f[1].w * dp1 + R.f[2].x * dp2 + R.f[2].y * dn0 + R.f[2].z * dn1 + R.f[2].w * dn2 + R.f[3].x * dr;
			if (INVDEPTH) D1 += R.f[3].y * di;
			const float D2 = R.f[1].z * dp0x3 + R.f[1].w * dp1x2 + R.f[2].x * dp2;
			A1 = last_alpha * D1p + (1.f - last_alpha) * A1;
			A2 = last_alpha * D2p + (1.f - last_alpha) * A2;
			D1p = D1; D2p = D2; last_alpha = alpha;
			const float bgterm = -T_final * inv_1ma * bg_dot_dpixel;
			const float dL_dalpha = selm0(ok, (D1 - A1) * T + bgterm);
			const float dL_dalpha_means2d = selm0(ok, (D2 - A2) * T + bgterm);
			v[GA_COLOR + 0] = w * dp0;
			v[GA_COLOR + 1] = w * dp1;
			v[GA_COLOR + 2] = w * dp2;
			v[GA_NORMAL + 0] = w * dn0;
			v[GA_NORMAL + 1] = w * dn1;
			v[GA_NORMAL + 2] = w * dn2;
			v[GA_REFL] = w * dr;
			v[GA_INVD] = INVDEPTH ? w * di : 0.f;
// ... 252 lines not shown
                                 const float* rotations, const float* cov3D_precomp, const float* viewmatrix, const float* projmatrix,
                                 const float* cam_pos, float tan_fovx, float tan_fovy, int prefiltered, float* out_color, float* out_normal_map,
                                 float* out_refl_strength_map, float* out_invdepth, int antialiasing, int* radii, int debug, void* stream_) {
	hipStream_t stream = (hipStream_t)stream_;
	if (!alloc || P < 0 || width <= 0 || height <= 0 || !background || !out_color || !out_normal_map || !out_refl_strength_map) {
		set_error("gsr_gauss_forward: invalid argument");
		return GSR_E_INVALID;
	}
	const size_t HW = (size_t)width * height;
	if (P == 0) {
		GSR_HIP_CHECK(hipMemsetAsync(out_color, 0, HW * 3 * 4, stream));
		GSR_HIP_CHECK(hipMemsetAsync(out_normal_map, 0, HW * 3 * 4, stream));
		GSR_HIP_CHECK(hipMemsetAsync(out_refl_strength_map, 0, HW * 4, stream));
		if (out_invdepth) GSR_HIP_CHECK(hipMemsetAsync(out_invdepth, 0, HW * 4, stream));
		return 0;
	}
	if (!means3D || !opacities || !normals || !refl_strengths || !viewmatrix || !projmatrix || !cam_pos || !radii ||
	    (!shs && !colors_precomp) || ((!scales || !rotations) && !cov3D_precomp)) {
		set_error("gsr_gauss_forward: missing required input pointer");
		return GSR_E_INVALID;
	}
	if (const int rc = check_sh_input("gsr_gauss_forward", D, M, shs); rc < 0) return rc;
	const int tiles_x = (width + 15) / 16, tiles_y = (height + 15) / 16;
	const int ntiles = tiles_x * tiles_y;
	GeomState geom; ImageState img;
	if (const int rc = forward_workspace(alloc, alloc_user, GAUSS_LAYOUT, P, HW, ntiles, &geom, &img); rc < 0) return rc;

	if (prefiltered) GSR_HIP_CHECK(hipMemsetAsync(geom.flags, 0, 4 * sizeof(int), stream));
	const RasterCam cam = make_cam(viewmatrix, projmatrix, cam_pos, width, height, tan_fovx, tan_fovy);
{ StageTimer st_(GSR_STAGE_PREPROCESS, stream); 	gauss_preprocess_kernel<<<(P + 255) / 256, 256, 0, stream>>>(P, D, M, means3D, scales, scale_modifier, rotations, opacities, shs, cov3D_precomp,
	                                                             colors_precomp, normals, refl_strengths, cam, radii, geom, tiles_x, tiles_y,
	                                                             prefiltered, antialiasing); }
	GSR_LAUNCH_CHECK(debug, stream);

	BinningState bin;
	const int R = run_binning(alloc, alloc_user, P, tiles_x, tiles_y, geom, img, &bin, prefiltered, debug, stream);
	if (R < 0) return R;

	const int nunits = (int)xcd_grid((uint32_t)ntiles * 4u);
	{
		StageTimer st_(GSR_STAGE_RENDER_FWD, stream);
		auto launch = [&](auto kern, auto pairs) {
			kern<<<nunits, 64, 0, stream>>>(img.ranges, img.tile_order, bin.point_list, width, height, tiles_x, ntiles, geom.rec, geom.bbox, option_cull(), background,
			                                img.final_T, img.n_contrib, out_color, out_normal_map, out_refl_strength_map, out_invdepth, bin.blend_mask, bin.mask_stride, pairs);
		};
		if (option_dev() & 2) {
			unsigned long long* word = dev_pair_counter();
			if (!word) { set_error("gsr_gauss_forward: no pair counter"); return GSR_E_HIP; }
			launch(out_invdepth ? gauss_render_fwd_wave_kernel<true, true> : gauss_render_fwd_wave_kernel<false, true>, PairCount<true>{word, option_dev() & 4});
		} else {
			launch(out_invdepth ? gauss_render_fwd_wave_kernel<true> : gauss_render_fwd_wave_kernel<false>, PairCount<false>{});
		}
	}
	GSR_LAUNCH_CHECK(debug, stream);
	return R;
}

extern "C" int gsr_gauss_backward_accum(int P, int D, int M, int R, const float* background, int width, int height, const float* means3D,
                                  const float* shs, const float* colors_precomp, const float* normals, const float* refl_strengths,
                                  const float* opacities, const float* scales, float scale_modifier, const float* rotations,
                                  const float* cov3D_precomp, const float* viewmatrix, const float* projmatrix, const float* cam_pos,
                                  float tan_fovx, float tan_fovy, const int* radii, void* geom_buffer, void* binning_buffer, void* image_buffer,
                                  const float* dL_dpix, const float* dL_dnormal_map, const float* dL_drefl_strength_map,
                                  const float* dL_invdepths, float* dL_dmean2D, float* dL_dmean2D_pixels, float* dL_dconic, float* dL_dopacity,
                                  float* dL_dcolor, float* dL_dnormals, float* dL_drefl_strengths, float* dL_dinvdepth, float* dL_dmean3D,
                                  float* dL_dcov3D, float* dL_dsh, float* dL_dscale, float* dL_drot, int antialiasing, int accumulate, int debug, void* stream_) {
	(void)colors_precomp; (void)normals; (void)refl_strengths;
	hipStream_t stream = (hipStream_t)stream_;
	const bool missing = !geom_buffer || !image_buffer || (R > 0 && !binning_buffer) || !dL_dpix || !dL_dnormal_map || !dL_drefl_strength_map ||
	    !dL_dmean2D_pixels || !dL_dopacity || (!shs && !dL_dcolor) || !dL_dnormals || !dL_drefl_strengths || !dL_dmean3D || (!scales && !dL_dcov3D) ||
	    !dL_dscale || !dL_drot || (shs && !dL_dsh) || (dL_invdepths && !dL_dinvdepth) || !radii || !means3D || !opacities;
	BackwardWorkspace w;
	if (const int rc = backward_prologue("gsr_gauss_backward", __func__, GAUSS_LAYOUT, P, M, R, width, height, missing, shs, dL_dsh, dL_drot, dL_dconic, "dL_dconic",
	                                     geom_buffer, binning_buffer, image_buffer, stream, &w); rc <= 0) return rc;
	const GeomState& geom = w.geom; const ImageState& img = w.img; const BinningState& bin = w.bin;
	const int tiles_x = w.tiles_x, ntiles = w.ntiles;
	if (R > 0) {
		const int nunits = (int)xcd_grid((uint32_t)ntiles * 4u);
		{
			StageTimer st_(GSR_STAGE_RENDER_BWD, stream);
			auto kern = dL_invdepths ? gauss_render_bwd_wave_kernel<true> : gauss_render_bwd_wave_kernel<false>;
			kern<<<nunits, 64, 0, stream>>>(img.ranges, img.tile_order, bin.point_list, width, height, tiles_x, ntiles, background, geom.rec, geom.bbox, option_cull(),
			                                img.final_T, img.n_contrib, dL_dpix, dL_dnormal_map, dL_drefl_strength_map, dL_invdepths, geom.acc, bin.blend_mask,
			                                bin.mask_stride);
		}
		GSR_LAUNCH_CHECK(debug, stream);
	}
	const RasterCam cam = make_cam(viewmatrix, projmatrix, cam_pos, width, height, tan_fovx, tan_fovy);
	const float* cov3D_ptr = cov3D_precomp;
{ StageTimer st_(GSR_STAGE_PREPROCESS_BWD, stream);
	auto kern = accumulate ? gauss_preprocess_bwd_kernel<true> : gauss_preprocess_bwd_kernel<false>;
	kern<<<(P + 255) / 256, 256, 0, stream>>>(P, D, M, means3D, radii, shs, geom.clamped, opacities, scales, rotations,
	                                                                 scale_modifier, cov3D_ptr, cam, geom.acc, dL_invdepths ? 1 : 0, antialiasing,
	                                                                 dL_dmean2D, dL_dmean2D_pixels, dL_dconic, dL_dopacity, dL_dcolor, dL_dnormals,
	                                                                 dL_drefl_strengths, dL_dinvdepth, dL_dmean3D, dL_dcov3D, dL_dsh, dL_dscale,
	                                                                 dL_drot); }
	GSR_LAUNCH_CHECK(debug, stream);
	return 0;
}

extern "C" int gsr_gauss_backward(int P, int D, int M, int R, const float* background, int width, int height, const float* means3D,
                                  const float* shs, const float* colors_precomp, const float* normals, const float* refl_strengths,
                                  const float* opacities, const float* scales, float scale_modifier, const float* rotations,
                                  const float* cov3D_precomp, const float* viewmatrix, const float* projmatrix, const float* cam_pos,
                                  float tan_fovx, float tan_fovy, const int* radii, void* geom_buffer, void* binning_buffer, void* image_buffer,
                                  const float* dL_dpix, const float* dL_dnormal_map, const float* dL_drefl_strength_map,
                                  const float* dL_invdepths, float* dL_dmean2D, float* dL_dmean2D_pixels, float* dL_dconic, float* dL_dopacity,
                                  float* dL_dcolor, float* dL_dnormals, float* dL_drefl_strengths, float* dL_dinvdepth, float* dL_dmean3D,
                                  float* dL_dcov3D, float* dL_dsh, float* dL_dscale, float* dL_drot, int antialiasing, int debug, void* stream_) {
	return gsr_gauss_backward_accum(P, D, M, R, background, width, height, means3D, shs, colors_precomp, normals, refl_strengths, opacities, scales,
	                                scale_modifier, rotations, cov3D_precomp, viewmatrix, projmatrix, cam_pos, tan_fovx, tan_fovy, radii, geom_buffer,
	                                binning_buffer, image_buffer, dL_dpix, dL_dnormal_map, dL_drefl_strength_map, dL_invdepths, dL_dmean2D,
	                                dL_dmean2D_pixels, dL_dconic, dL_dopacity, dL_dcolor, dL_dnormals, dL_drefl_strengths, dL_dinvdepth, dL_dmean3D,
	                                dL_dcov3D, dL_dsh, dL_dscale, dL_drot, antialiasing, 0, debug, stream_);
}
```

### gaussian-splatting-reflection_amd/csrc/gsr_internal.hpp

```cpp
#pragma once
#include <cstring>
#include <cstdint>
#include <cstdio>
#include <hip/hip_runtime.h>
#include "../../include/gsr_hip.h"

#define GSR_TILE 16
#define GSR_TILE_PIX 256

namespace gsr {

void set_error(const char* fmt, ...);
#define GSR_HIP_CHECK(expr)                                                                       \
	do {                                                                                          \
		hipError_t _e = (expr);                                                                   \
		if (_e != hipSuccess) {                                                                   \
			gsr::set_error("%s failed: %s (%s:%d)", #expr, hipGetErrorString(_e), __FILE__, __LINE__); \
			return GSR_E_HIP;                                                                     \
		}                                                                                         \
	} while (0)
#define GSR_LAUNCH_CHECK(debug, stream)                                  \
	do {                                                                 \
		GSR_HIP_CHECK(hipGetLastError());                                \
		if (debug) GSR_HIP_CHECK(hipStreamSynchronize(stream));          \
	} while (0)

static inline bool misaligned16(const void* p) { return (reinterpret_cast<uintptr_t>(p) & 15u) != 0; }
#define GSR_REQUIRE_ALIGNED16_IN(func, ptr, what)                                                             \
	do {                                                                                                      \
		if ((ptr) && gsr::misaligned16(ptr)) {                                                                \
			gsr::set_error("%s: %s must be 16-byte aligned (float4 accesses); got %p", func, what, (const void*)(ptr)); \
			return GSR_E_INVALID;                                                                             \
		}                                                                                                     \
	} while (0)
#define GSR_REQUIRE_ALIGNED16(ptr, what) GSR_REQUIRE_ALIGNED16_IN(__func__, ptr, what)

struct StageTimer {
	int stage;
	hipStream_t stream;
	void* rec;
	StageTimer(int stage, hipStream_t stream);
	~StageTimer();
};

struct Carver {
	char* base;
	size_t off;
	explicit Carver(void* b) : base((char*)b), off(0) {}
	template <class T> T* take(size_t count) {
		off = (off + 255) & ~(size_t)255;
		T* p = base ? (T*)(base + off) : nullptr;
		off += count * sizeof(T);
		return p;
	}
	size_t size() const { return (off + 255) & ~(size_t)255; }
};

struct GeomState {
	float* depths;
	uint32_t* rect;
	uint32_t* tiles_touched;
	uint32_t* point_offsets;
	uint8_t* clamped;
	float4* rec;
	float4* bbox;
	float* aux;
	float* acc;
	int* flags;
	uint32_t* depth_sorted;
	unsigned long long* order;
	unsigned long long* emit_state;
	size_t emit_state_bytes;
	void* scan_temp;
	size_t scan_temp_bytes;
	void* depth_sort_temp;
	size_t depth_sort_bytes, depth_sort_clear;
};
struct ImageState {
	uint2* ranges;
	float* final_T;
	uint32_t* n_contrib;
	uint32_t* tile_order;
};
struct BinningState {
	uint32_t* point_list;
	unsigned long long* blend_mask;
	size_t mask_stride;
	uint32_t* tile_keys;
	uint32_t* tile_keys_unsorted;
	uint32_t* vals_unsorted;
	void* sort_temp;
	size_t sort_temp_bytes;
};

#define S_REC_F4 5
#define S_ACC_F 20
#define G_REC_F4 4
#define G_ACC_F 16
struct WorkspaceLayout {
	int rec_f4, aux_floats, acc_floats;
	int planes_T, planes_n;
	constexpr WorkspaceLayout inference() const { return {rec_f4, aux_floats, 0, 0, 0}; }
};
constexpr WorkspaceLayout SURFEL_LAYOUT{S_REC_F4, 0, S_ACC_F, 3, 2};
constexpr WorkspaceLayout GAUSS_LAYOUT{G_REC_F4, 0, G_ACC_F, 1, 1};

GeomState carve_geom(void* buf, size_t P, const WorkspaceLayout& layout, size_t* total);
ImageState carve_image(void* buf, size_t HW, size_t tiles, const WorkspaceLayout& layout, size_t* total);
BinningState carve_binning(void* buf, size_t R, size_t tiles, size_t sort_temp_bytes, size_t* total, bool blend_masks = true);
int forward_workspace(gsr_alloc_fn alloc, void* alloc_user, const WorkspaceLayout& layout, size_t P, size_t HW, size_t tiles, GeomState* geom,
                      ImageState* img);

static inline int check_sh_input(const char* entry, int D, int M, const float* shs) {
	if (D < 0 || D > 3 || (shs && (D + 1) * (D + 1) > M)) { set_error("%s: SH degree %d not supported with M=%d", entry, D, M); return GSR_E_INVALID; }
	if (shs && ((M * 3) & 3) == 0 && misaligned16(shs)) {
		set_error("%s: shs (rows of a multiple of 16 bytes) must be 16-byte aligned (float4 accesses); got %p", entry, (const void*)shs);
		return GSR_E_INVALID;
	}
	return 0;
}

struct RasterCam {
	const float* view;
	const float* proj;
	const float* campos;
	int W, H;
	float tan_fovx, tan_fovy, focal_x, focal_y;
};
static inline RasterCam make_cam(const float* view, const float* proj, const float* campos, int W, int H, float tan_fovx, float tan_fovy) {
	RasterCam c;
	c.view = view; c.proj = proj; c.campos = campos; c.W = W; c.H = H;
	c.tan_fovx = tan_fovx; c.tan_fovy = tan_fovy;
	c.focal_y = H / (2.0f * tan_fovy);
	c.focal_x = W / (2.0f * tan_fovx);
	return c;
}

struct BackwardWorkspace { GeomState geom; ImageState img; BinningState bin; int tiles_x, ntiles; };
static inline int backward_prologue(const char* entry, const char* func, const WorkspaceLayout& layout, int P, int M, int R, int width, int height,
                                    bool missing_pointer, const float* shs, const float* dL_dsh, const float* dL_drot, const float* also_aligned,
                                    const char* also_what, void* geom_buffer, void* binning_buffer, void* image_buffer, hipStream_t stream,
                                    BackwardWorkspace* w) {
	if (P < 0 || R < 0 || width <= 0 || height <= 0) { set_error("%s: invalid size", entry); return GSR_E_INVALID; }
	if (P == 0) return 0;
	if (missing_pointer) { set_error("%s: missing required pointer", entry); return GSR_E_INVALID; }
	if (shs && ((M * 3) & 3) == 0) GSR_REQUIRE_ALIGNED16_IN(func, shs, "shs (rows of a multiple of 16 bytes)");
	if (shs && ((M * 3) & 3) == 0) GSR_REQUIRE_ALIGNED16_IN(func, dL_dsh, "dL_dsh");
	GSR_REQUIRE_ALIGNED16_IN(func, dL_drot, "dL_drot");
	GSR_REQUIRE_ALIGNED16_IN(func, also_aligned, also_what);
	w->tiles_x = (width + 15) / 16;
	w->ntiles = w->tiles_x * ((height + 15) / 16);
	w->geom = carve_geom(geom_buffer, P, layout, nullptr);
	w->img = carve_image(image_buffer, (size_t)width * height, w->ntiles, layout, nullptr);
	w->bin = carve_binning(binning_buffer, R, w->ntiles, 0, nullptr);
	GSR_HIP_CHECK(hipMemsetAsync(w->geom.acc, 0, (size_t)P * layout.acc_floats * sizeof(float), stream));
	return 1;
}

int option_cull();
int option_dev();
unsigned long long* dev_pair_counter();
size_t sort_temp_bytes(size_t R, int end_bit);
int run_tile_order(const ImageState& img, size_t tiles, hipStream_t stream);
uint32_t higher_msb(uint32_t n);

int run_binning(gsr_alloc_fn alloc, void* alloc_user, int P, int tiles_x, int tiles_y, const GeomState& geom,
                const ImageState& img, BinningState* out_binning, int prefiltered, int debug, hipStream_t stream, bool blend_masks = true);

int side_gate_wait(hipStream_t stream);
int refl_sort_keys_early(uint32_t L, int width, int height, float* scratch, size_t scratch_floats, const uint32_t* sort_keys, int async, bool gated,
                         hipStream_t stream);

}

#ifdef __HIPCC__
namespace gsr {

__device__ __forceinline__ int f2i(float v) { return (int)v; }

__device__ __forceinline__ void get_rect(float px, float py, int max_radius, int gx, int gy, uint32_t& x0, uint32_t& y0,
                                         uint32_t& x1, uint32_t& y1) {
	const float r = (float)max_radius;
	x0 = (uint32_t)min(gx, max(0, f2i((px - r) / 16.0f)));
	y0 = (uint32_t)min(gy, max(0, f2i((py - r) / 16.0f)));
	x1 = (uint32_t)min(gx, max(0, f2i((px + r + 15.0f) / 16.0f)));
	y1 = (uint32_t)min(gy, max(0, f2i((py + r + 15.0f) / 16.0f)));
}

#define GSR_DPP1(CTRL, i) "v_add_f32_dpp %" #i ", %" #i ", %" #i " " CTRL "\n\t"
#define GSR_DPP4(CTRL) GSR_DPP1(CTRL, 0) GSR_DPP1(CTRL, 1) GSR_DPP1(CTRL, 2) GSR_DPP1(CTRL, 3)
#define GSR_SHR1 "row_shr:1 row_mask:0xf bank_mask:0xf bound_ctrl:0"
#define GSR_SHR2 "row_shr:2 row_mask:0xf bank_mask:0xf bound_ctrl:0"
#define GSR_SHR4 "row_shr:4 row_mask:0xf bank_mask:0xf bound_ctrl:0"
#define GSR_SHR8 "row_shr:8 row_mask:0xf bank_mask:0xf bound_ctrl:0"
#define GSR_BC15 "row_bcast:15 row_mask:0xa bank_mask:0xf"
#define GSR_BC31 "row_bcast:31 row_mask:0xc bank_mask:0xf"
__device__ __forceinline__ void wave_sum4(float* v) {
	asm volatile("s_nop 1\n\t" GSR_DPP4(GSR_SHR1) GSR_DPP4(GSR_SHR2) GSR_DPP4(GSR_SHR4) GSR_DPP4(GSR_SHR8) GSR_DPP4(GSR_BC15) GSR_DPP4(GSR_BC31)
	             : "+v"(v[0]), "+v"(v[1]), "+v"(v[2]), "+v"(v[3]));
}

#define GSR_Q1(CTRL, i) "v_add_f32_dpp %" #i ", %" #i ", %" #i " " CTRL " row_mask:0xf bank_mask:0xf\n\t"
#define GSR_DPPB(CTRL, BANK, dst, src) "v_add_f32_dpp %" #dst ", %" #src ", %" #src " " CTRL " row_mask:0xf bank_mask:" BANK "\n\t"
#define GSR_L1(CTRL, d, a, b) GSR_DPPB(CTRL, "0x3", d, a) GSR_DPPB(CTRL, "0xc", d, b)
__device__ __forceinline__ void row_reduce20(const float* v, float* z) {
	float p0, q0, p1, q1, p2, q2, p3, q3, p4, q4;
	asm volatile("s_nop 1\n\t" GSR_L1("row_mirror", 0, 6, 7) GSR_L1("row_mirror", 1, 8, 9) GSR_L1("row_mirror", 2, 10, 11)
	             GSR_L1("row_mirror", 3, 12, 13) GSR_L1("row_mirror", 4, 14, 15) GSR_L1("row_mirror", 5, 16, 17)
	             : "=&v"(p0), "=&v"(q0), "=&v"(p1), "=&v"(q1), "=&v"(p2), "=&v"(q2)
	             : "v"(v[0]), "v"(v[1]), "v"(v[2]), "v"(v[3]), "v"(v[4]), "v"(v[5]), "v"(v[6]), "v"(v[7]), "v"(v[8]), "v"(v[9]), "v"(v[10]), "v"(v[11]));
	asm volatile("s_nop 1\n\t" GSR_L1("row_mirror", 0, 4, 5) GSR_L1("row_mirror", 1, 6, 7) GSR_L1("row_mirror", 2, 8, 9) GSR_L1("row_mirror", 3, 10, 11)
	             : "=&v"(p3), "=&v"(q3), "=&v"(p4), "=&v"(q4)
	             : "v"(v[12]), "v"(v[13]), "v"(v[14]), "v"(v[15]), "v"(v[16]), "v"(v[17]), "v"(v[18]), "v"(v[19]));
#define GSR_L2(d, a, b) GSR_DPPB("row_half_mirror", "0x5", d, a) GSR_DPPB("row_half_mirror", "0xa", d, b)
#define GSR_QA(CTRL) GSR_Q1(CTRL, 0) GSR_Q1(CTRL, 1) GSR_Q1(CTRL, 2) GSR_Q1(CTRL, 3) GSR_Q1(CTRL, 4)
	asm volatile("s_nop 1\n\t" GSR_L2(0, 5, 6) GSR_L2(1, 7, 8) GSR_L2(2, 9, 10) GSR_L2(3, 11, 12) GSR_L2(4, 13, 14)
	             GSR_QA("quad_perm:[2,3,0,1]") GSR_QA("quad_perm:[1,0,3,2]")
	             : "=&v"(z[0]), "=&v"(z[1]), "=&v"(z[2]), "=&v"(z[3]), "=&v"(z[4])
	             : "v"(p0), "v"(q0), "v"(p1), "v"(q1), "v"(p2), "v"(q2), "v"(p3), "v"(q3), "v"(p4), "v"(q4));
}
__device__ __forceinline__ void row_reduce16(const float* v, float* z) {
	float p0, q0, p1, q1, p2, q2, p3, q3;
	asm volatile("s_nop 1\n\t" GSR_L1("row_mirror", 0, 8, 9) GSR_L1("row_mirror", 1, 10, 11) GSR_L1("row_mirror", 2, 12, 13) GSR_L1("row_mirror", 3, 14, 15)
	             GSR_L1("row_mirror", 4, 16, 17) GSR_L1("row_mirror", 5, 18, 19) GSR_L1("row_mirror", 6, 20, 21) GSR_L1("row_mirror", 7, 22, 23)
	             : "=&v"(p0), "=&v"(q0), "=&v"(p1), "=&v"(q1), "=&v"(p2), "=&v"(q2), "=&v"(p3), "=&v"(q3)
	             : "v"(v[0]), "v"(v[1]), "v"(v[2]), "v"(v[3]), "v"(v[4]), "v"(v[5]), "v"(v[6]), "v"(v[7]), "v"(v[8]), "v"(v[9]), "v"(v[10]), "v"(v[11]),
	               "v"(v[12]), "v"(v[13]), "v"(v[14]), "v"(v[15]));
#define GSR_QB(CTRL) GSR_Q1(CTRL, 0) GSR_Q1(CTRL, 1) GSR_Q1(CTRL, 2) GSR_Q1(CTRL, 3)
	asm volatile("s_nop 1\n\t" GSR_L2(0, 4, 5) GSR_L2(1, 6, 7) GSR_L2(2, 8, 9) GSR_L2(3, 10, 11)
	             GSR_QB("quad_perm:[2,3,0,1]") GSR_QB("quad_perm:[1,0,3,2]")
	             : "=&v"(z[0]), "=&v"(z[1]), "=&v"(z[2]), "=&v"(z[3])
	             : "v"(p0), "v"(q0), "v"(p1), "v"(q1), "v"(p2), "v"(q2), "v"(p3), "v"(q3));
}
__device__ __forceinline__ int sub_px(int lane) { return ((lane >> 4) & 1) * 4 + (lane & 3); }
__device__ __forceinline__ int sub_py(int lane) { return (lane >> 5) * 4 + ((lane >> 2) & 3); }
__device__ __forceinline__ void wave_lds_sync() {
	__builtin_amdgcn_fence(__ATOMIC_RELEASE, "wavefront");
	__builtin_amdgcn_wave_barrier();
	__builtin_amdgcn_fence(__ATOMIC_ACQUIRE, "wavefront");
}
template <int N, bool ACC>
__device__ __forceinline__ void wave_store_rows(float* lds, const float* v, float* __restrict__ out, int nrows, int lane) {
#pragma unroll
	for (int k = 0; k < N; k++) lds[k * 65 + lane] = v[k];
	wave_lds_sync();
#pragma unroll
	for (int j = 0; j < N; j++) {
		const int e = lane + 64 * j, r = e / N, k = e - r * N;
		if (r < nrows) {
			const float x = lds[k * 65 + r];
			if (ACC) {
				if (x != 0.f) out[e] += x;
// ... 160 lines not shown
```

### gaussian-splatting-reflection_amd/csrc/gsr_sort.hpp

```cpp
#pragma once
#include <hip/hip_runtime.h>
#include <rocprim/device/device_radix_sort.hpp>
#include <rocprim/iterator/counting_iterator.hpp>
#include <rocprim/rocprim_version.hpp>

#if ROCPRIM_VERSION / 100 == 4002
#define GSR_ONESWEEP_DRIVER 1
#else
#define GSR_ONESWEEP_DRIVER 0
#endif

namespace gsr {

int option_sort_driver();

using SortOffset = unsigned int;
constexpr size_t ONESWEEP_MAX_ITEMS = (size_t)1 << 30;

#if GSR_ONESWEEP_DRIVER
using SortBlockId = rocprim::detail::block_id_wrapper<unsigned int, true>;
using SortLookback = rocprim::detail::onesweep_lookback_state;
static_assert(sizeof(SortLookback) == 4, "onesweep_lookback_state is expected to be one 32-bit word (flag in the top two bits)");
static_assert(SortLookback::EMPTY == 0, "a zero-filled look-back state must mean EMPTY: the driver clears the states with zeros");

// ... 33 lines not shown

struct OnesweepLayout { unsigned places, blocks; size_t o_next, o_lookback, lookback_pass, o_ids, cleared; };
static inline size_t sort_up256(size_t b) { return (b + 255) & ~(size_t)255; }
template <unsigned BS, unsigned IPT, unsigned BITS>
OnesweepLayout onesweep_layout(unsigned size, unsigned begin_bit, unsigned end_bit) {
	constexpr size_t radix = (size_t)1 << BITS;
	OnesweepLayout l;
	l.places = (end_bit - begin_bit + BITS - 1) / BITS;
	l.blocks = (size + BS * IPT - 1) / (BS * IPT);
	l.o_next = sort_up256(radix * l.places * sizeof(SortOffset));
	l.o_lookback = l.o_next + sort_up256(radix * sizeof(SortOffset));
	l.lookback_pass = sort_up256(radix * (l.blocks ? l.blocks : 1) * sizeof(SortLookback));
	l.o_ids = l.o_lookback + l.lookback_pass * l.places;
	l.cleared = l.o_ids + sort_up256((size_t)l.places * 64);
	return l;
}

template <unsigned BS, unsigned IPT, unsigned BITS, class ValuesIn, class Value>
hipError_t onesweep_sort_pairs(void* temp, size_t& bytes, const uint32_t* keys_in, uint32_t* keys_out, ValuesIn values_in, Value* values_out, size_t size_,
                               unsigned begin_bit, unsigned end_bit, hipStream_t stream, bool pre_cleared, const SortOffset* ext_counts,
                               hipEvent_t before_last_pass) {
	static_assert(sizeof(Value) == 4 || sizeof(Value) == 8, "4- or 8-byte values");
	constexpr unsigned radix = 1u << BITS, items_per_block = BS * IPT;
	if (size_ >= ONESWEEP_MAX_ITEMS || end_bit <= begin_bit) return hipErrorInvalidValue;
	const unsigned size = (unsigned)size_;
	const OnesweepLayout l = onesweep_layout<BS, IPT, BITS>(size, begin_bit, end_bit);
	const unsigned places = l.places, blocks = l.blocks, full_blocks = size % items_per_block == 0 ? blocks : blocks - 1;
	const size_t o_vals_tmp = l.cleared + sort_up256((size_t)size * 4), total = o_vals_tmp + sort_up256((size_t)size * sizeof(Value));
	if (temp == nullptr) { bytes = total; return hipSuccess; }
	if (bytes < total) return hipErrorInvalidValue;
	if (size == 0) return hipSuccess;
	char* base = static_cast<char*>(temp);
	SortOffset* digits = reinterpret_cast<SortOffset*>(base);
	SortOffset* next = reinterpret_cast<SortOffset*>(base + l.o_next);
	uint32_t* keys_tmp = reinterpret_cast<uint32_t*>(base + l.cleared);
	Value* values_tmp = reinterpret_cast<Value*>(base + o_vals_tmp);

	if (!pre_cleared) {
		hipError_t e = hipMemsetAsync(base, 0, l.cleared, stream);
		if (e != hipSuccess) return e;
	}
	const SortOffset* counts = ext_counts;
	if (counts == nullptr) {
		constexpr unsigned HIPT = IPT < 16 ? 16 : IPT, hist_items = BS * HIPT;
		const unsigned hist_blocks = (size + hist_items - 1) / hist_items;
		const unsigned hist_full = size % hist_items == 0 ? hist_blocks : hist_blocks - 1;
		sort_histogram_kernel<BS, HIPT, BITS><<<hist_blocks, BS, 0, stream>>>(keys_in, digits, size, hist_full, begin_bit, end_bit);
		counts = digits;
	}

	bool to_output = (places - 1) % 2 == 0, from_input = true;
	unsigned place = 0;
	for (unsigned bit = begin_bit; bit < end_bit; bit += BITS, ++place) {
		const unsigned current_bits = (end_bit - bit) < BITS ? (end_bit - bit) : BITS;
		SortLookback* lookback = reinterpret_cast<SortLookback*>(base + l.o_lookback + l.lookback_pass * place);
		SortBlockId block_id = SortBlockId::create(base + l.o_ids + (size_t)place * 64);
		const SortOffset* d_in = counts + (size_t)place * radix;
		uint32_t* k_out = to_output ? keys_out : keys_tmp;
		Value* v_out = to_output ? values_out : values_tmp;
		if (before_last_pass != nullptr && place + 1 == places) {
			hipError_t e = hipEventRecord(before_last_pass, stream);
			if (e != hipSuccess) return e;
		}
		if (from_input) {
			sort_pass_kernel<BS, IPT, BITS, ValuesIn, Value><<<blocks, BS, 0, stream>>>(keys_in, k_out, values_in, v_out, size, d_in, next, lookback, bit,
			                                                                            current_bits, full_blocks, block_id);
		} else {
			const uint32_t* k_in = to_output ? keys_tmp : keys_out;
			const Value* v_in = to_output ? values_tmp : values_out;
			sort_pass_kernel<BS, IPT, BITS, const Value*, Value><<<blocks, BS, 0, stream>>>(k_in, k_out, v_in, v_out, size, d_in, next, lookback, bit,
			                                                                                current_bits, full_blocks, block_id);
		}
		from_input = false;
		to_output = !to_output;
	}
	return hipGetLastError();
}
#endif

__device__ __forceinline__ void sort_clear_region(void* ptr, size_t bytes, size_t thread, size_t threads) {
	uint4* p = static_cast<uint4*>(ptr);
	for (size_t i = thread; i < bytes / 16; i += threads) p[i] = make_uint4(0u, 0u, 0u, 0u);
}

template <class T> const T* sort_values_in(T* p) { return p; }
template <class It> It sort_values_in(It it) { return it; }

template <unsigned BS, unsigned IPT, unsigned BITS, class PublicConfig = rocprim::default_config>
struct RadixSort {
	template <class KeysIn, class ValuesIn, class Value>
	static size_t temp_bytes(KeysIn keys_in, ValuesIn values_in, Value* values_out, size_t n, unsigned end_bit) {
		size_t own = 0, pub = 0;
#if GSR_ONESWEEP_DRIVER
		(void)onesweep_sort_pairs<BS, IPT, BITS>(nullptr, own, keys_in, nullptr, sort_values_in(values_in), values_out, n, 0u, end_bit, nullptr, false, nullptr, nullptr);
#endif
		(void)rocprim::radix_sort_pairs<PublicConfig>(nullptr, pub, keys_in, (uint32_t*)nullptr, values_in, values_out, n, 0u, end_bit, nullptr, false);
		return own > pub ? own : pub;
	}
	static size_t cleared_bytes(size_t n, unsigned end_bit) {
#if GSR_ONESWEEP_DRIVER
		if (n < ONESWEEP_MAX_ITEMS && end_bit > 0) return onesweep_layout<BS, IPT, BITS>((unsigned)n, 0u, end_bit).cleared;
#endif
		return 0;
	}
	template <class KeysIn, class ValuesIn, class Value>
	static hipError_t pairs(void* temp, size_t bytes, KeysIn keys_in, uint32_t* keys_out, ValuesIn values_in, Value* values_out, size_t n, unsigned end_bit,
	                        hipStream_t stream, bool pre_cleared = false, const SortOffset* ext_counts = nullptr, hipEvent_t before_last_pass = nullptr) {
#if GSR_ONESWEEP_DRIVER
		if (option_sort_driver() && n < ONESWEEP_MAX_ITEMS)
			return onesweep_sort_pairs<BS, IPT, BITS>(temp, bytes, keys_in, keys_out, sort_values_in(values_in), values_out, n, 0u, end_bit, stream, pre_cleared,
			                                          ext_counts, before_last_pass);
#endif
		hipError_t e = rocprim::radix_sort_pairs<PublicConfig>(temp, bytes, keys_in, keys_out, values_in, values_out, n, 0u, end_bit, stream, false);
		if (e == hipSuccess && before_last_pass != nullptr) e = hipEventRecord(before_last_pass, stream);
		return e;
	}
};

}
```

### gaussian-splatting-reflection_amd/csrc/gsr_surfel.hip

```cpp
#include <type_traits>
#include "gsr_internal.hpp"
#include "gsr_tile_walk.hpp"
#include "gsr_sort.hpp"
#include "gsr_math.hpp"
#include "gsr_refl.hpp"

namespace gsr {

#define SA_COLOR 0
#define SA_REFL 3
#define SA_NORMAL 4
#define SA_OPAC 7
#define SA_T 8
#define SA_MEAN2D 17

#define S_NEAR 0.2f
#define S_FAR 100.0f
#define S_FILTER_INV_SQ 2.0f

__device__ __forceinline__ M3 quat_to_rotmat(const float* __restrict__ q, float& w, float& x, float& y, float& z) {
#pragma clang fp contract(off)
	const float s = 1.0f / sqrtf(q[3] * q[3] + q[0] * q[0] + q[1] * q[1] + q[2] * q[2]);
	w = q[0] * s; x = q[1] * s; y = q[2] * s; z = q[3] * s;
	return m3_make(1.f - 2.f * (y * y + z * z), 2.f * (x * y + w * z), 2.f * (x * z - w * y), 2.f * (x * y - w * z),
// ... 80 lines not shown
                      const float* __restrict__ rotations, const float* __restrict__ opacities, const float* __restrict__ shs,
                      const float* __restrict__ transMat_precomp, const float* __restrict__ colors_precomp, const float* __restrict__ refl,
                      const uint8_t* __restrict__ env_scope_mask, const RasterCam& cam, int* __restrict__ radii, const GeomState& g, int gx, int gy,
                      int prefiltered, float* __restrict__ gaussian_weights, float4* o) {
#pragma clang fp contract(off)
	radii[idx] = 0;
	if constexpr (TRAIN) gaussian_weights[idx] = 0.f;
	g.tiles_touched[idx] = 0;
	reinterpret_cast<uint2*>(g.rect)[idx] = make_uint2(0u, 0u);
	g.depths[idx] = __int_as_float(0x7f7fffff);
	const float mx = means[3 * idx], my = means[3 * idx + 1], mz = means[3 * idx + 2];
	const float* vm = cam.view;
	const float pvx = vm[0] * mx + vm[4] * my + vm[8] * mz + vm[12];
	const float pvy = vm[1] * mx + vm[5] * my + vm[9] * mz + vm[13];
	const float pvz = vm[2] * mx + vm[6] * my + vm[10] * mz + vm[14];
	if (pvz <= 0.2f) {
		if (prefiltered) g.flags[0] = 1;
		return false;
	}
	M3 T;
	F3 normal;
	if (transMat_precomp == nullptr) {
		compute_transmat(mx, my, mz, scales + 2 * idx, scale_modifier, rotations + 4 * idx, cam, T, normal);
	} else {
#pragma unroll
		for (int c = 0; c < 3; c++)
#pragma unroll
			for (int r = 0; r < 3; r++) T.m[c][r] = transMat_precomp[9 * idx + 3 * c + r];
		normal = f3(0.0f, 0.0f, 1.0f);
	}
	const float cosv = -((pvx * normal.x) + (pvy * normal.y) + (pvz * normal.z));
	if (cosv == 0) return false;
	const float multiplier = cosv > 0 ? 1.f : -1.f;
	normal = f3(multiplier * normal.x, multiplier * normal.y, multiplier * normal.z);
	const float cutoff = 3.0f;
	const float t0 = cutoff * cutoff, t1 = cutoff * cutoff, t2 = -1.0f;
	const float d = t0 * (T.m[2][0] * T.m[2][0]) + t1 * (T.m[2][1] * T.m[2][1]) + t2 * (T.m[2][2] * T.m[2][2]);
	if (d == 0.0f) return false;
	const float inv_d = 1 / d;
	const float f0 = inv_d * t0, f1 = inv_d * t1, f2 = inv_d * t2;
	const float pxi = f0 * (T.m[0][0] * T.m[2][0]) + f1 * (T.m[0][1] * T.m[2][1]) + f2 * (T.m[0][2] * T.m[2][2]);
	const float pyi = f0 * (T.m[1][0] * T.m[2][0]) + f1 * (T.m[1][1] * T.m[2][1]) + f2 * (T.m[1][2] * T.m[2][2]);
	const float h0x = pxi * pxi - (f0 * (T.m[0][0] * T.m[0][0]) + f1 * (T.m[0][1] * T.m[0][1]) + f2 * (T.m[0][2] * T.m[0][2]));
	const float h0y = pyi * pyi - (f0 * (T.m[1][0] * T.m[1][0]) + f1 * (T.m[1][1] * T.m[1][1]) + f2 * (T.m[1][2] * T.m[1][2]));
	const float ex = sqrtf(fmaxf(1e-4f, h0x)), ey = sqrtf(fmaxf(1e-4f, h0y));
	const float radius = ceilf(fmaxf(fmaxf(ex, ey), cutoff * (float)0.707106));
	uint32_t x0, y0, x1, y1;
	get_rect(pxi, pyi, f2i(radius), gx, gy, x0, y0, x1, y1);
	if ((x1 - x0) * (y1 - y0) == 0) return false;

	float cr, cg, cb;
	if (colors_precomp == nullptr) {
		const float dx = mx - cam.campos[0], dy = my - cam.campos[1], dz = mz - cam.campos[2];
		const float len = sqrtf(dx * dx + dy * dy + dz * dz);
		ShRow s;
		load_sh(shs, idx, M, (D + 1) * (D + 1), s);
		const F3 c = sh_eval(D, s, dx / len, dy / len, dz / len);
		if constexpr (TRAIN) g.clamped[idx] = (uint8_t)((c.x < 0 ? 1 : 0) | (c.y < 0 ? 2 : 0) | (c.z < 0 ? 4 : 0));
		cr = fmaxf(c.x, 0.0f); cg = fmaxf(c.y, 0.0f); cb = fmaxf(c.z, 0.0f);
	} else {
		cr = colors_precomp[3 * idx]; cg = colors_precomp[3 * idx + 1]; cb = colors_precomp[3 * idx + 2];
	}
	g.depths[idx] = pvz;
	radii[idx] = f2i(radius);
	g.rect[2 * idx] = x0 | (y0 << 16);
	g.rect[2 * idx + 1] = x1 | (y1 << 16);
	const float maskv = (env_scope_mask != nullptr && env_scope_mask[idx]) ? 1.0f : 0.0f;
	surfel_cull_record(T, pxi, pyi, opacities[idx], o[5], o[6]);
	float4* rec = o;
	rec[0] = make_float4(pxi, pyi, T.m[0][0], T.m[1][0]);
	rec[1] = make_float4(T.m[0][1], T.m[1][1], T.m[0][2], T.m[1][2]);
	rec[2] = make_float4(T.m[2][0], T.m[2][1], T.m[2][2], opacities[idx]);
	rec[3] = make_float4(normal.x, normal.y, normal.z, refl[idx]);
	rec[4] = make_float4(cr, cg, cb, maskv);
	g.tiles_touched[idx] = (y1 - y0) * (x1 - x0);
	return true;
}

#define S_OUT_F4 7
struct CubemapInterleave {
	const float* cubemap;
	float4* rgba;
	uint32_t ntex, LL;
};
template <bool TRAIN>
__global__ void __launch_bounds__(256)
surfel_preprocess_kernel(int P, int D, int M, const float* __restrict__ means, const float* __restrict__ scales, float scale_modifier,
                         const float* __restrict__ rotations, const float* __restrict__ opacities, const float* __restrict__ shs,
                         const float* __restrict__ transMat_precomp, const float* __restrict__ colors_precomp,
                         const float* __restrict__ refl, const uint8_t* __restrict__ env_scope_mask, RasterCam cam, int* __restrict__ radii,
                         GeomState g, int gx, int gy, int prefiltered, float* __restrict__ gaussian_weights, CubemapInterleave ci) {
	const int idx = blockIdx.x * 256 + threadIdx.x;
	for (uint32_t t = (uint32_t)idx; t < ci.ntex; t += gridDim.x * 256u) {
		const uint32_t f = t / ci.LL, r = t - f * ci.LL;
		const float* c = ci.cubemap + (size_t)f * 3 * ci.LL + r;
		ci.rgba[t] = make_float4(c[0], c[ci.LL], c[2 * (size_t)ci.LL], 0.f);
	}
	sort_clear_region(g.depth_sort_temp, g.depth_sort_clear, (size_t)idx, (size_t)gridDim.x * 256u);
	sort_clear_region(g.emit_state, g.emit_state_bytes, (size_t)idx, (size_t)gridDim.x * 256u);
	if (idx == 0) { g.flags[1] = 0; g.flags[2] = 0; g.flags[3] = 0; }
	__shared__ float4 s_out[4][S_REC_F4 * 65];
	const int lane = threadIdx.x & 63;
	float4* so = s_out[threadIdx.x >> 6];
	float4 o[S_OUT_F4];
#pragma unroll
	for (int k = 0; k < S_OUT_F4; k++) o[k] = make_float4(0.f, 0.f, 0.f, 0.f);
	bool live = false;
	if (idx < P)
		live = surfel_preprocess_one<TRAIN>(idx, D, M, means, scales, scale_modifier, rotations, opacities, shs, transMat_precomp, colors_precomp, refl,
		                             env_scope_mask, cam, radii, g, gx, gy, prefiltered, gaussian_weights, o);
	if (__ballot(live) == 0ull) return;
	const int g0 = idx - lane;
	const int ng = min(64, P - g0);
	wave_store_rows4<S_REC_F4, false>(so, o, g.rec + (size_t)g0 * S_REC_F4, S_REC_F4, 0, ng, lane);
	wave_store_rows4<2, false>(so, o + S_REC_F4, g.bbox + (size_t)g0 * 2, 2, 0, ng, lane);
}

typedef float v2f __attribute__((ext_vector_type(2)));
__device__ __forceinline__ v2f mk2(float a, float b) { v2f r; r.x = a; r.y = b; return r; }

struct SurfelRec : TileRec<S_REC_F4> {
	__device__ __forceinline__ v2f xy() const { return mk2(f[0].x, f[0].y); }
	__device__ __forceinline__ v2f TuvX() const { return mk2(f[0].z, f[0].w); }
	__device__ __forceinline__ v2f TuvY() const { return mk2(f[1].x, f[1].y); }
	__device__ __forceinline__ v2f TuvZ() const { return mk2(f[1].z, f[1].w); }
	__device__ __forceinline__ v2f Twxy() const { return mk2(f[2].x, f[2].y); }
	__device__ __forceinline__ float Twz() const { return f[2].z; }
	__device__ __forceinline__ float opac() const { return f[2].w; }
	__device__ __forceinline__ v2f nxy() const { return mk2(f[3].x, f[3].y); }
	__device__ __forceinline__ float nz() const { return f[3].z; }
	__device__ __forceinline__ float refl() const { return f[3].w; }
	__device__ __forceinline__ v2f rg() const { return mk2(f[4].x, f[4].y); }
	__device__ __forceinline__ float b() const { return f[4].z; }
	__device__ __forceinline__ float mask() const { return f[4].w; }
};

#ifndef GSR_BWD_WPE
#define GSR_BWD_WPE 4
#endif
#ifndef GSR_BWD_LIST
#define GSR_BWD_LIST 1
#endif
#ifndef GSR_BWD_UNROLL
#define GSR_BWD_UNROLL 1
#endif
#ifdef GSR_FWD_WPE
#define GSR_FWD_ATTR __attribute__((amdgpu_waves_per_eu(GSR_FWD_WPE, GSR_FWD_WPE)))
#else
#define GSR_FWD_ATTR
#endif

struct SurfelFwdPix {
	float T, C2, M2, distortion, median_depth, median_contributor, maskacc;
	v2f Crg, Nxy, NzR, DM;
	uint32_t last_contributor;
};

template <bool TRAIN>
__device__ __forceinline__ lmask surfel_fwd_pair(const SurfelRec& R, const v2f pix, uint32_t contributor, bool med_live, SurfelFwdPix& st,
                                                 lmask& done, float& wq, bool& grazed) {
	float sx, sy, rho3d, depth, alpha, rho2d;
	{
#pragma clang fp contract(off)
		const v2f Tw = R.Twxy();
		const v2f X = pix * Tw.x - R.TuvX();
		const v2f Y = pix * Tw.y - R.TuvY();
		const v2f Z = pix * R.Twz() - R.TuvZ();
		const v2f a = Y * Z.yx;
		const v2f b = Z * X.yx;
		const v2f c = X * Y.yx;
		const float ppx = a.x - a.y, ppy = b.x - b.y, pz = c.x - c.y;
		const lmask unstable = LMASK(fabsf(pz) < 1e-4f);
		if (__builtin_expect(unstable == 0ull, 1)) {
			const float inv = div_nr(1.0f, pz);
			sx = ppx * inv; sy = ppy * inv;
			rho3d = sx * sx + sy * sy;
		} else {
			if constexpr (TRAIN) grazed = true;
			const float inv = div_nr(1.0f, selm(unstable, 1.0f, pz));
			sx = selm(unstable, 0.f, ppx * inv); sy = selm(unstable, 0.f, ppy * inv);
			rho3d = selm(unstable, 1e8f, sx * sx + sy * sy);
		}
		const v2f d = R.xy() - pix;
// ... 448 lines not shown
					const lmask em = (0xFFull << (8 * e)) & todo;
					if (em == 0ull) continue;
					const lmask cc = c | em;
					if (c != 0ull && __popcll(m0 & cc) + __popcll(m1 & cc) + __popcll(m2 & cc) + __popcll(m3 & cc) > S_CAP) break;
					c = cc;
				}
			}
			const lmask c0 = m0 & todo & c, c1 = m1 & todo & c, c2 = m2 & todo & c, c3 = m3 & todo & c, call = any & todo & c;
			todo &= ~c;
			const int n0 = __popcll(c0), n1 = __popcll(c1), n2 = __popcll(c2), n3 = __popcll(c3);
			const int nmax = __builtin_amdgcn_readfirstlane(max(max(n0, n1), max(n2, n3)));
			const int nent = __popcll(call);
			if ((call >> lane) & 1ull) {
				const uint32_t s0 = ((c0 >> lane) & 1ull) ? (uint32_t)__popcll(c0 & gt) : (uint32_t)(S_CAP + 1);
				const uint32_t s1 = ((c1 >> lane) & 1ull) ? (uint32_t)(n0 + __popcll(c1 & gt)) : (uint32_t)(S_CAP + 1);
				const uint32_t s2 = ((c2 >> lane) & 1ull) ? (uint32_t)(n0 + n1 + __popcll(c2 & gt)) : (uint32_t)(S_CAP + 1);
				const uint32_t s3 = ((c3 >> lane) & 1ull) ? (uint32_t)(n0 + n1 + n2 + __popcll(c3 & gt)) : (uint32_t)(S_CAP + 1);
				const int k = __popcll(call & lt);
				s_cw[k] = s0 | (s1 << 6) | (s2 << 12) | (s3 << 18) | ((uint32_t)lane << 24);
#if GSR_BWD_LIST
				if ((c0 >> lane) & 1ull) s_list[s0] = (uint8_t)lane;
				if ((c1 >> lane) & 1ull) s_list[s1] = (uint8_t)lane;
				if ((c2 >> lane) & 1ull) s_list[s2] = (uint8_t)lane;
				if ((c3 >> lane) & 1ull) s_list[s3] = (uint8_t)lane;
#endif
			}
			__syncthreads();
#if !GSR_BWD_LIST
			unsigned long long left = __builtin_bitreverse64(row == 0 ? c0 : (row == 1 ? c1 : (row == 2 ? c2 : c3)));
#else
			const int nrow = row == 0 ? n0 : (row == 1 ? n1 : (row == 2 ? n2 : n3));
#endif
			const uint32_t rowbase = (uint32_t)(row == 0 ? 0 : (row == 1 ? n0 : (row == 2 ? n0 + n1 : n0 + n1 + n2)));
			uint32_t myslot = rowbase * (S_ACC_F * 4u) + slab_lane;
#pragma unroll GSR_BWD_UNROLL
			for (int t = 0; t < nmax; t++) {
#if !GSR_BWD_LIST
				const uint32_t lo = (uint32_t)left, hi = (uint32_t)(left >> 32);
				const lmask valid = LMASK((lo | hi) != 0u);
				const uint32_t tz = min(ffbl_raw(lo), ffbl_raw(hi) | 32u);
				const uint32_t j = selmu(valid, 63u - tz, jany);
				left &= left - 1ull;
#else
				const lmask valid = LMASK(t < nrow);
				const uint32_t j = selmu(valid, (uint32_t)s_list[min(rowbase + (uint32_t)t, 63u)], jany);
#endif
				const float4* q = reinterpret_cast<const float4*>(reinterpret_cast<const char*>(s_rec) + __umul24(j, S_REC_F4 * 16u));
				const SurfelRec R{q[0], q[1], q[2], q[3], q[4]};
				float v[S_ACC_F];
				v[S_ACC_F - 1] = 0.f;
				surfel_bwd_pair(st, R, pixv, b * WBATCH + (int)j, inside_m & valid, v);
				float z[5];
				row_reduce20(v, z);
				float* slab = reinterpret_cast<float*>(reinterpret_cast<char*>(s_slab) + selmu(valid, myslot, (uint32_t)(S_CAP * S_ACC_F * 4) + slab_lane));
				myslot += S_ACC_F * 4u;
#pragma unroll
				for (int g = 0; g < 5; g++) slab[4 * g] = z[g];
			}
			__syncthreads();
#pragma unroll 1
			for (int k0 = 0; k0 < nent; k0 += 3) {
				const uint32_t k = (uint32_t)k0 + fl_k;
				if (fl_on && k < (uint32_t)nent) {
					const uint32_t w = s_cw[k];
					const uint32_t eid = __float_as_uint(s_rec[(w >> 24) * S_REC_F4 + 4].w);
					const char* base = slab_b + fl_d * 4u;
					const float a0 = *reinterpret_cast<const float*>(base + (w & 0x3Fu) * (S_ACC_F * 4u));
					const float a1 = *reinterpret_cast<const float*>(base + ((w >> 6) & 0x3Fu) * (S_ACC_F * 4u));
					const float a2 = *reinterpret_cast<const float*>(base + ((w >> 12) & 0x3Fu) * (S_ACC_F * 4u));
					const float a3 = *reinterpret_cast<const float*>(base + ((w >> 18) & 0x3Fu) * (S_ACC_F * 4u));
					if (!(dev_flags & 1)) atomicAdd(fl_acc + (size_t)eid * S_ACC_F, (a0 + a1) + (a2 + a3));
				}
			}
			__syncthreads();
		}
	}
}

__global__ void __launch_bounds__(64) __attribute__((amdgpu_waves_per_eu(GSR_BWD_WPE, GSR_BWD_WPE)))
surfel_render_bwd_rows_kernel(const uint2* __restrict__ ranges, const uint32_t* __restrict__ tile_order, const uint32_t* __restrict__ point_list, int W, int H, int tiles_x, int ntiles,
                              const float* __restrict__ bg, const float4* __restrict__ rec, int dev_flags, const float* __restrict__ final_Ts,
                              const uint32_t* __restrict__ n_contrib, const float* __restrict__ dL_dpixels, const float* __restrict__ dL_depths,
                              const float* __restrict__ dL_drefl_map, const float* __restrict__ dL_dnormal_extra, float* __restrict__ acc,
                              const unsigned long long* __restrict__ blend_mask) {
	surfel_render_bwd_rows_body(ranges, tile_order, point_list, W, H, tiles_x, ntiles, bg, rec, dev_flags, final_Ts, n_contrib, dL_dpixels, dL_depths,
	                            dL_drefl_map, dL_dnormal_extra, acc, blend_mask);
}

__device__ __forceinline__ void quat_vjp(float w, float x, float y, float z, const M3& v_R, float* v_quat) {
	v_quat[0] = 2.f * (x * (v_R.m[1][2] - v_R.m[2][1]) + y * (v_R.m[2][0] - v_R.m[0][2]) + z * (v_R.m[0][1] - v_R.m[1][0]));
	v_quat[1] = 2.f * (-2.f * x * (v_R.m[1][1] + v_R.m[2][2]) + y * (v_R.m[0][1] + v_R.m[1][0]) + z * (v_R.m[0][2] + v_R.m[2][0]) + w * (v_R.m[1][2] - v_R.m[2][1]));
	v_quat[2] = 2.f * (x * (v_R.m[0][1] + v_R.m[1][0]) - 2.f * y * (v_R.m[0][0] + v_R.m[2][2]) + z * (v_R.m[1][2] + v_R.m[2][1]) + w * (v_R.m[2][0] - v_R.m[0][2]));
	v_quat[3] = 2.f * (x * (v_R.m[0][2] + v_R.m[2][0]) + y * (v_R.m[1][2] + v_R.m[2][1]) - 2.f * z * (v_R.m[0][0] + v_R.m[1][1]) + w * (v_R.m[0][1] - v_R.m[1][0]));
}

template <bool ACC>
__global__ void __launch_bounds__(256)
surfel_preprocess_bwd_kernel(int P, int D, int M, const float* __restrict__ means, const int* __restrict__ radii, const float* __restrict__ shs,
                             const uint8_t* __restrict__ clamped, const float* __restrict__ scales, const float* __restrict__ rotations,
                             const float4* __restrict__ rec, RasterCam cam, const float* __restrict__ acc, float* __restrict__ dL_dmean2D,
                             float* __restrict__ dL_dnormal, float* __restrict__ dL_dopacity, float* __restrict__ dL_dcolor,
                             float* __restrict__ dL_drefl, float* __restrict__ dL_dmean3D, float* __restrict__ dL_dtransMat,
                             float* __restrict__ dL_dsh, float* __restrict__ dL_dscale, float* __restrict__ dL_drot) {
	__shared__ __attribute__((aligned(16))) float s_tile[4][1368];
	const int lane = threadIdx.x & 63;
	float* tile = s_tile[threadIdx.x >> 6];
	const int idx_raw = blockIdx.x * 256 + threadIdx.x;
	const int g0 = idx_raw - lane, nrows = min(64, P - g0);
	if (nrows <= 0) return;
	const bool in_range = idx_raw < P;
	const int idx = in_range ? idx_raw : P - 1;
	const float4* a4 = reinterpret_cast<const float4*>(acc + (size_t)idx * S_ACC_F);
	const float4 a0 = a4[0], a1 = a4[1], a2 = a4[2], a3 = a4[3], a4v = a4[4];
	const float gcol[3] = {a0.x, a0.y, a0.z};
	const float gnrm[3] = {a1.x, a1.y, a1.z};
	float dT[9] = {a2.x, a2.y, a2.z, -a2.w, -a3.x, -a3.y, a3.z, a3.w, a4v.x};
	const float gm2x = a4v.y, gm2y = a4v.z;
	if (in_range) {
		put<ACC>(dL_drefl + idx, a0.w);
		put<ACC>(dL_dopacity + idx, a1.w);
	}

	float dmean[3] = {0.f, 0.f, 0.f}, dscale[2] = {0.f, 0.f}, drot[4] = {0.f, 0.f, 0.f, 0.f};
	float out_m2x = gm2x, out_m2y = gm2y;
	float dTout[9];
#pragma unroll
	for (int i = 0; i < 9; i++) dTout[i] = dT[i];
	const bool visible = radii[idx] > 0;
	const float mx = means[3 * idx], my = means[3 * idx + 1], mz = means[3 * idx + 2];
	if (visible) {
		const int Wb = f2i(cam.focal_x * cam.tan_fovx * 2);
		const int Hb = f2i(cam.focal_y * cam.tan_fovy * 2);
		const bool precomp = (scales == nullptr);
		M3 T;
		F3 normal = f3(0.f, 0.f, 0.f);
		P34 Pm;
		M3 R;
		float qw = 0, qx = 0, qy = 0, qz = 0, sc0 = 0, sc1 = 0;
		const float4* rc = rec + (size_t)idx * S_REC_F4;
		if (precomp) {
			const float4 r0 = rc[0], r1 = rc[1], r2 = rc[2];
			T = m3_make(r0.z, r1.x, r1.z, r0.w, r1.y, r1.w, r2.x, r2.y, r2.z);
		} else {
			R = quat_to_rotmat(rotations + 4 * idx, qw, qx, qy, qz);
			sc0 = scales[2 * idx]; sc1 = scales[2 * idx + 1];
			const float L0[3] = {R.m[0][0] * sc0, R.m[0][1] * sc0, R.m[0][2] * sc0};
			const float L1[3] = {R.m[1][0] * sc1, R.m[1][1] * sc1, R.m[1][2] * sc1};
			Pm = make_P(cam.proj, Wb, Hb);
#pragma unroll
			for (int j = 0; j < 3; j++) {
				T.m[j][0] = L0[0] * Pm.m[j][0] + L0[1] * Pm.m[j][1] + L0[2] * Pm.m[j][2];
				T.m[j][1] = L1[0] * Pm.m[j][0] + L1[1] * Pm.m[j][1] + L1[2] * Pm.m[j][2];
				T.m[j][2] = mx * Pm.m[j][0] + my * Pm.m[j][1] + mz * Pm.m[j][2] + Pm.m[j][3];
			}
			const float* vm = cam.view;
			const float nx = R.m[2][0], ny = R.m[2][1], nz = R.m[2][2];
			normal = f3(vm[0] * nx + vm[4] * ny + vm[8] * nz, vm[1] * nx + vm[5] * ny + vm[9] * nz, vm[2] * nx + vm[6] * ny + vm[10] * nz);
		}
		M3 dL_dT = m3_make(dT[0], dT[1], dT[2], dT[3], dT[4], dT[5], dT[6], dT[7], dT[8]);
		bool early = false;
		if (gm2x != 0 || gm2y != 0) {
			const float tv[3] = {9.0f, 9.0f, -1.0f};
			const float d = tv[0] * (T.m[2][0] * T.m[2][0]) + tv[1] * (T.m[2][1] * T.m[2][1]) + tv[2] * (T.m[2][2] * T.m[2][2]);
			const float invd = 1.0f / d;
			float fv[3], dL_df[3], dT3[3];
#pragma unroll
			for (int r = 0; r < 3; r++) fv[r] = tv[r] * invd;
// ... 55 lines not shown
		if (M == 16) {
			float w[16];
			F3 grgb = f3(0.f, 0.f, 0.f);
#pragma unroll
			for (int k = 0; k < 16; k++) w[k] = 0.f;
			if (visible && (gcol[0] != 0.f || gcol[1] != 0.f || gcol[2] != 0.f)) {
				ShRow s;
				load_sh(shs, idx, M, (D + 1) * (D + 1), s);
				const F3 dir = f3(mx - cam.campos[0], my - cam.campos[1], mz - cam.campos[2]);
				grgb = f3(gcol[0], gcol[1], gcol[2]);
				const F3 dm = sh_backward_weights(D, s, dir, clamped[idx], grgb, w);
				dmean[0] += dm.x; dmean[1] += dm.y; dmean[2] += dm.z;
			}
			float4* sh_out = reinterpret_cast<float4*>(dL_dsh) + (size_t)g0 * 12;
#pragma unroll
			for (int t = 0; t < 3; t++) {
				const float4 q4[4] = {sh_row_f4(4 * t, w, grgb), sh_row_f4(4 * t + 1, w, grgb), sh_row_f4(4 * t + 2, w, grgb), sh_row_f4(4 * t + 3, w, grgb)};
				wave_store_rows4<4, ACC>(reinterpret_cast<float4*>(tile), q4, sh_out, 12, 4 * t, nrows, lane);
			}
		} else if (in_range) {
			if (visible) {
				ShRow s;
				load_sh(shs, idx, M, (D + 1) * (D + 1), s);
				const F3 dir = f3(mx - cam.campos[0], my - cam.campos[1], mz - cam.campos[2]);
				const F3 dm = sh_backward<ACC>(idx, D, M, s, dir, clamped[idx], f3(gcol[0], gcol[1], gcol[2]), dL_dsh);
				dmean[0] += dm.x; dmean[1] += dm.y; dmean[2] += dm.z;
			} else if (!ACC) {
				float* out = dL_dsh + (size_t)idx * M * 3;
				for (int q = 0; q < M * 3; q++) out[q] = 0.f;
			}
		}
	}
	const float m2d[3] = {out_m2x, out_m2y, 0.f};
	if (dL_dcolor != nullptr) wave_store_rows<3, false>(tile, gcol, dL_dcolor + (size_t)g0 * 3, nrows, lane);
	if (dL_dnormal != nullptr) wave_store_rows<3, false>(tile, gnrm, dL_dnormal + (size_t)g0 * 3, nrows, lane);
	wave_store_rows<3, false>(tile, m2d, dL_dmean2D + (size_t)g0 * 3, nrows, lane);
	wave_store_rows<3, ACC>(tile, dmean, dL_dmean3D + (size_t)g0 * 3, nrows, lane);
	if (dL_dtransMat != nullptr) wave_store_rows<9, false>(tile, dTout, dL_dtransMat + (size_t)g0 * 9, nrows, lane);
	if (in_range) {
		put<ACC>(dL_dscale + 2 * idx, dscale[0]); put<ACC>(dL_dscale + 2 * idx + 1, dscale[1]);
		float4* rq = reinterpret_cast<float4*>(dL_drot) + idx;
		if (ACC) {
			if (drot[0] != 0.f || drot[1] != 0.f || drot[2] != 0.f || drot[3] != 0.f) {
				const float4 r0 = *rq;
				*rq = make_float4(r0.x + drot[0], r0.y + drot[1], r0.z + drot[2], r0.w + drot[3]);
			}
		} else {
			*rq = make_float4(drot[0], drot[1], drot[2], drot[3]);
		}
	}
}

}

using namespace gsr;

static int check_refl_descriptor(const char* entry, const gsr_refl_forward* refl) {
	if (!refl) return 0;
	if (!refl->cam || !refl->cubemap || !refl->fail_value || refl->L == 0 || !refl->cubemap_rgba || ((uintptr_t)refl->cubemap_rgba & 15) != 0 ||
	    !refl->out_final || !refl->out_refl_color || !refl->out_normal_world) {
		set_error("%s: incomplete reflection descriptor (cam, cubemap, fail_value, L, 16-byte aligned cubemap_rgba and the three outputs are required)", entry);
		return GSR_E_INVALID;
	}
	if ((size_t)6 * refl->L * refl->L >= 0xFFFFFFFFull) { set_error("%s: cubemap too large", entry); return GSR_E_INVALID; }
	return 0;
}
static int check_surfel_inputs(const char* entry, int P, int D, int M, const float* means3D, const float* shs, const float* colors_precomp,
                               const float* refl_strengths, const float* opacities, const float* scales, const float* rotations,
                               const float* transMat_precomp, const float* viewmatrix, const float* projmatrix, const float* cam_pos, const int* radii) {
	if (P == 0) return 0;
	if (!means3D || !opacities || !refl_strengths || !viewmatrix || !projmatrix || !cam_pos || !radii || (!shs && !colors_precomp) ||
	    ((!scales || !rotations) && !transMat_precomp)) {
		set_error("%s: missing required input pointer", entry);
		return GSR_E_INVALID;
	}
	return check_sh_input(entry, D, M, shs);
}

static int early_key_sort(const gsr_refl_forward* refl, int width, int height, int R, hipStream_t stream) {
	if (!refl || !refl->sort_keys || !refl->scratch) return 0;
	return refl_sort_keys_early(refl->L, width, height, refl->scratch, refl->scratch_floats, refl->sort_keys, refl->async_sort, R > 0, stream);
}

template <bool TRAIN>
static int surfel_forward(gsr_alloc_fn alloc, void* alloc_user, int P, int D, int M, const float* background, int width, int height,
                          const float* means3D, const uint8_t* env_scope_mask, const float* shs, const float* colors_precomp,
                          const float* refl_strengths, const float* opacities, const float* scales, float scale_modifier,
                          const float* rotations, const float* transMat_precomp, const float* viewmatrix, const float* projmatrix,
                          const float* cam_pos, float tan_fovx, float tan_fovy, int prefiltered, float* out_color, float* out_others,
                          float* out_alpha, float* out_normal_view, float* out_refl_strength_map, int* radii, float* gaussian_weights,
                          const gsr_refl_forward* refl, int debug, hipStream_t stream) {
	const size_t HW = (size_t)width * height;
	int R = 0;
	if (P == 0) {
		float* normal = TRAIN ? out_others + 2 * HW : out_normal_view;
		if (!normal) {
			normal = static_cast<float*>(alloc(alloc_user, GSR_BUF_IMAGE, HW * 3 * 4));
			if (!normal) { set_error("workspace allocation failed (%zu bytes)", HW * 3 * 4); return GSR_E_ALLOC; }
		}
		GSR_HIP_CHECK(hipMemsetAsync(out_color, 0, HW * 3 * 4, stream));
		if (TRAIN) {
			GSR_HIP_CHECK(hipMemsetAsync(out_others, 0, HW * 8 * 4, stream));
		} else {
			GSR_HIP_CHECK(hipMemsetAsync(out_alpha, 0, HW * 4, stream));
			GSR_HIP_CHECK(hipMemsetAsync(normal, 0, HW * 3 * 4, stream));
		}
		GSR_HIP_CHECK(hipMemsetAsync(out_refl_strength_map, 0, HW * 4, stream));
		if (refl && gsr_deferred_reflection_forward_keys(normal, out_color, out_refl_strength_map, refl->cam, refl->cubemap, refl->fail_value, refl->L,
		                                                 width, height, refl->out_final, refl->out_refl_color, refl->out_normal_world, refl->cubemap_rgba,
		                                                 refl->sort_keys, stream) < 0)
			return GSR_E_HIP;
	} else {
		const int tiles_x = (width + 15) / 16, tiles_y = (height + 15) / 16;
		const int ntiles = tiles_x * tiles_y;
		GeomState geom; ImageState img;
		if (const int rc = forward_workspace(alloc, alloc_user, TRAIN ? SURFEL_LAYOUT : SURFEL_LAYOUT.inference(), P, HW, ntiles, &geom, &img); rc < 0) return rc;

		if (prefiltered) GSR_HIP_CHECK(hipMemsetAsync(geom.flags, 0, 4 * sizeof(int), stream));
		const RasterCam cam = make_cam(viewmatrix, projmatrix, cam_pos, width, height, tan_fovx, tan_fovy);
		CubemapInterleave ci{nullptr, nullptr, 0u, 1u};
		SurfelReflFwd rf{};
		if (refl) {
			ci = CubemapInterleave{refl->cubemap, reinterpret_cast<float4*>(refl->cubemap_rgba), 6u * refl->L * refl->L, refl->L * refl->L};
			rf = SurfelReflFwd{refl->cam, refl->cubemap, reinterpret_cast<const float4*>(refl->cubemap_rgba), refl->fail_value, (int)refl->L, 6u * refl->L * refl->L,
			                   refl->out_final, refl->out_refl_color, refl->out_normal_world, refl->sort_keys};
		}
	{ StageTimer st_(GSR_STAGE_PREPROCESS, stream); 	surfel_preprocess_kernel<TRAIN><<<(P + 255) / 256, 256, 0, stream>>>(P, D, M, means3D, scales, scale_modifier, rotations, opacities, shs,
		                                                                     transMat_precomp, colors_precomp, refl_strengths, env_scope_mask, cam, radii, geom,
		                                                                     tiles_x, tiles_y, prefiltered, gaussian_weights, ci); }
		GSR_LAUNCH_CHECK(debug, stream);

		BinningState bin;
		R = run_binning(alloc, alloc_user, P, tiles_x, tiles_y, geom, img, &bin, prefiltered, debug, stream, TRAIN);
		if (R < 0) return R;

	{ StageTimer st_(GSR_STAGE_RENDER_FWD, stream);
		const int nunits = (int)xcd_grid((uint32_t)ntiles * 4u);
		const auto args = [&] { if constexpr (TRAIN) return rf; else return SurfelEvalFwd{rf, out_alpha, out_normal_view}; }();
		auto launch = [&](auto render, auto pairs) {
			render<<<nunits, 64, 0, stream>>>(img.ranges, img.tile_order, bin.point_list, width, height, tiles_x, ntiles, geom.rec, geom.bbox, option_cull(),
			                                  background, TRAIN ? img.final_T : nullptr, TRAIN ? img.n_contrib : nullptr, out_color, out_others,
			                                  out_refl_strength_map, gaussian_weights, bin.blend_mask, bin.mask_stride, args, pairs);
		};
		if (option_dev() & 2) {
			unsigned long long* word = dev_pair_counter();
			if (!word) { set_error("gsr_surfel_forward: no pair counter"); return GSR_E_HIP; }
			launch(refl ? surfel_render_fwd_wave_kernel<true, TRAIN, true> : surfel_render_fwd_wave_kernel<false, TRAIN, true>, PairCount<true>{word, option_dev() & 4});
		} else {
			launch(refl ? surfel_render_fwd_wave_kernel<true, TRAIN> : surfel_render_fwd_wave_kernel<false, TRAIN>, PairCount<false>{});
		} }
		GSR_LAUNCH_CHECK(debug, stream);
	}
	if (const int rc = TRAIN ? early_key_sort(refl, width, height, R, stream) : 0; rc < 0) return rc;
	return R;
}

extern "C" int gsr_surfel_forward_refl(gsr_alloc_fn alloc, void* alloc_user, int P, int D, int M, const float* background, int width, int height,
                                  const float* means3D, const uint8_t* env_scope_mask, const float* shs, const float* colors_precomp,
                                  const float* refl_strengths, const float* opacities, const float* scales, float scale_modifier,
                                  const float* rotations, const float* transMat_precomp, const float* viewmatrix, const float* projmatrix,
                                  const float* cam_pos, float tan_fovx, float tan_fovy, int prefiltered, float* out_color, float* out_others,
                                  float* out_refl_strength_map, int* radii, float* gaussian_weights, const gsr_refl_forward* refl, int debug,
                                  void* stream_) {
	if (!alloc || P < 0 || width <= 0 || height <= 0 || !background || !out_color || !out_others || !out_refl_strength_map) {
		set_error("gsr_surfel_forward: invalid argument");
		return GSR_E_INVALID;
	}
	if (P > 0 && !gaussian_weights) { set_error("gsr_surfel_forward: missing required input pointer"); return GSR_E_INVALID; }
	if (const int rc = check_refl_descriptor("gsr_surfel_forward_refl", refl); rc < 0) return rc;
	if (const int rc = check_surfel_inputs("gsr_surfel_forward", P, D, M, means3D, shs, colors_precomp, refl_strengths, opacities, scales, rotations,
	                                       transMat_precomp, viewmatrix, projmatrix, cam_pos, radii); rc < 0) return rc;
	return surfel_forward<true>(alloc, alloc_user, P, D, M, background, width, height, means3D, env_scope_mask, shs, colors_precomp, refl_strengths,
	                            opacities, scales, scale_modifier, rotations, transMat_precomp, viewmatrix, projmatrix, cam_pos, tan_fovx, tan_fovy,
	                            prefiltered, out_color, out_others, nullptr, nullptr, out_refl_strength_map, radii, gaussian_weights, refl, debug,
	                            (hipStream_t)stream_);
}

extern "C" int gsr_surfel_forward(gsr_alloc_fn alloc, void* alloc_user, int P, int D, int M, const float* background, int width, int height,
                                  const float* means3D, const uint8_t* env_scope_mask, const float* shs, const float* colors_precomp,
                                  const float* refl_strengths, const float* opacities, const float* scales, float scale_modifier,
                                  const float* rotations, const float* transMat_precomp, const float* viewmatrix, const float* projmatrix,
                                  const float* cam_pos, float tan_fovx, float tan_fovy, int prefiltered, float* out_color, float* out_others,
                                  float* out_refl_strength_map, int* radii, float* gaussian_weights, int debug, void* stream_) {
	return gsr_surfel_forward_refl(alloc, alloc_user, P, D, M, background, width, height, means3D, env_scope_mask, shs, colors_precomp, refl_strengths, opacities,
	                               scales, scale_modifier, rotations, transMat_precomp, viewmatrix, projmatrix, cam_pos, tan_fovx, tan_fovy, prefiltered, out_color,
	                               out_others, out_refl_strength_map, radii, gaussian_weights, nullptr, debug, stream_);
}

extern "C" int gsr_surfel_forward_eval(gsr_alloc_fn alloc, void* alloc_user, int P, int D, int M, const float* background, int width, int height,
                                       const float* means3D, const float* shs, const float* colors_precomp, const float* refl_strengths,
                                       const float* opacities, const float* scales, float scale_modifier, const float* rotations,
                                       const float* transMat_precomp, const float* viewmatrix, const float* projmatrix, const float* cam_pos,
                                       float tan_fovx, float tan_fovy, int prefiltered, float* out_color, float* out_alpha,
                                       float* out_normal_view, float* out_refl_strength_map, int* radii, const gsr_refl_forward* refl,
                                       int debug, void* stream_) {
	if (!alloc || P < 0 || width <= 0 || height <= 0 || !background || !out_color || !out_alpha || !out_refl_strength_map) {
		set_error("gsr_surfel_forward_eval: invalid argument (alloc, P >= 0, width, height, background, out_color, out_alpha, out_refl_strength_map)");
		return GSR_E_INVALID;
	}
	if (!out_normal_view && !refl) { set_error("gsr_surfel_forward_eval: out_normal_view may be NULL only with refl"); return GSR_E_INVALID; }
	if (refl && (refl->sort_keys || refl->scratch)) {
		set_error("gsr_surfel_forward_eval: refl->sort_keys and refl->scratch must be NULL (the eval forward has no backward)");
		return GSR_E_INVALID;
	}
	if (const int rc = check_refl_descriptor("gsr_surfel_forward_eval", refl); rc < 0) return rc;
	if (const int rc = check_surfel_inputs("gsr_surfel_forward_eval", P, D, M, means3D, shs, colors_precomp, refl_strengths, opacities, scales, rotations,
	                                       transMat_precomp, viewmatrix, projmatrix, cam_pos, radii); rc < 0) return rc;
	return surfel_forward<false>(alloc, alloc_user, P, D, M, background, width, height, means3D, nullptr, shs, colors_precomp, refl_strengths, opacities,
	                             scales, scale_modifier, rotations, transMat_precomp, viewmatrix, projmatrix, cam_pos, tan_fovx, tan_fovy, prefiltered,
	                             out_color, nullptr, out_alpha, out_normal_view, out_refl_strength_map, radii, nullptr, refl, debug, (hipStream_t)stream_);
}

extern "C" int gsr_surfel_backward_ex(int P, int D, int M, int R, const float* background, int width, int height, const float* means3D,
                                   const float* shs, const float* colors_precomp, const float* refl_strengths, const float* scales,
                                   float scale_modifier, const float* rotations, const float* transMat_precomp, const float* viewmatrix,
                                   const float* projmatrix, const float* cam_pos, float tan_fovx, float tan_fovy, const int* radii,
                                   void* geom_buffer, void* binning_buffer, void* image_buffer, const float* dL_dpix, const float* dL_dothers,
                                   const float* dL_drefl_strength_map, float* dL_dmean2D, float* dL_dnormal, float* dL_dopacity, float* dL_dcolor,
                                   float* dL_drefl_strengths, float* dL_dmean3D, float* dL_dtransMat, float* dL_dsh, float* dL_dscale,
                                   float* dL_drot, int accumulate, const float* dL_dnormal_extra, int debug, void* stream_) {
	(void)colors_precomp; (void)refl_strengths; (void)scale_modifier; (void)transMat_precomp;
	hipStream_t stream = (hipStream_t)stream_;
	const bool missing = !geom_buffer || !image_buffer || (R > 0 && !binning_buffer) || !dL_dpix || !dL_dothers || !dL_drefl_strength_map || !dL_dmean2D ||
	    !dL_dopacity || !dL_drefl_strengths || !dL_dmean3D || !dL_dscale || !dL_drot || (!shs && !dL_dcolor) || (!scales && !dL_dtransMat) ||
	    (shs && !dL_dsh) || !radii || !means3D;
	BackwardWorkspace w;
	if (const int rc = backward_prologue("gsr_surfel_backward", __func__, SURFEL_LAYOUT, P, M, R, width, height, missing, shs, dL_dsh, dL_drot, nullptr, nullptr,
	                                     geom_buffer, binning_buffer, image_buffer, stream, &w); rc <= 0) return rc;
	const GeomState& geom = w.geom; const ImageState& img = w.img; const BinningState& bin = w.bin;
	const int tiles_x = w.tiles_x, ntiles = w.ntiles;
	if (R > 0) {
		{ const int rc = side_gate_wait(stream); if (rc < 0) return rc; }
{ StageTimer st_(GSR_STAGE_RENDER_BWD, stream);
		const int nunits = (int)xcd_grid((uint32_t)ntiles * 4u);
		surfel_render_bwd_rows_kernel<<<nunits, 64, 0, stream>>>(img.ranges, img.tile_order, bin.point_list, width, height, tiles_x, ntiles, background, geom.rec,
		                                                         option_dev(), img.final_T, img.n_contrib, dL_dpix, dL_dothers, dL_drefl_strength_map, dL_dnormal_extra,
		                                                         geom.acc, bin.blend_mask); }
		GSR_LAUNCH_CHECK(debug, stream);
	}
	const RasterCam cam = make_cam(viewmatrix, projmatrix, cam_pos, width, height, tan_fovx, tan_fovy);
{ StageTimer st_(GSR_STAGE_PREPROCESS_BWD, stream);
	auto kern = accumulate ? surfel_preprocess_bwd_kernel<true> : surfel_preprocess_bwd_kernel<false>;
	kern<<<(P + 255) / 256, 256, 0, stream>>>(P, D, M, means3D, radii, shs, geom.clamped, scales, rotations, geom.rec, cam, geom.acc, dL_dmean2D, dL_dnormal,
	                                          dL_dopacity, dL_dcolor, dL_drefl_strengths, dL_dmean3D, dL_dtransMat, dL_dsh, dL_dscale, dL_drot); }
	GSR_LAUNCH_CHECK(debug, stream);
	return 0;
}

extern "C" int gsr_surfel_backward(int P, int D, int M, int R, const float* background, int width, int height, const float* means3D,
                                   const float* shs, const float* colors_precomp, const float* refl_strengths, const float* scales,
                                   float scale_modifier, const float* rotations, const float* transMat_precomp, const float* viewmatrix,
                                   const float* projmatrix, const float* cam_pos, float tan_fovx, float tan_fovy, const int* radii,
                                   void* geom_buffer, void* binning_buffer, void* image_buffer, const float* dL_dpix, const float* dL_dothers,
                                   const float* dL_drefl_strength_map, float* dL_dmean2D, float* dL_dnormal, float* dL_dopacity, float* dL_dcolor,
                                   float* dL_drefl_strengths, float* dL_dmean3D, float* dL_dtransMat, float* dL_dsh, float* dL_dscale,
                                   float* dL_drot, int debug, void* stream_) {
	return gsr_surfel_backward_ex(P, D, M, R, background, width, height, means3D, shs, colors_precomp, refl_strengths, scales, scale_modifier, rotations,
	                              transMat_precomp, viewmatrix, projmatrix, cam_pos, tan_fovx, tan_fovy, radii, geom_buffer, binning_buffer, image_buffer,
	                              dL_dpix, dL_dothers, dL_drefl_strength_map, dL_dmean2D, dL_dnormal, dL_dopacity, dL_dcolor, dL_drefl_strengths, dL_dmean3D,
	                              dL_dtransMat, dL_dsh, dL_dscale, dL_drot, 0, nullptr, debug, stream_);
}

extern "C" int gsr_surfel_backward_accum(int P, int D, int M, int R, const float* background, int width, int height, const float* means3D,
                                   const float* shs, const float* colors_precomp, const float* refl_strengths, const float* scales,
                                   float scale_modifier, const float* rotations, const float* transMat_precomp, const float* viewmatrix,
                                   const float* projmatrix, const float* cam_pos, float tan_fovx, float tan_fovy, const int* radii,
                                   void* geom_buffer, void* binning_buffer, void* image_buffer, const float* dL_dpix, const float* dL_dothers,
                                   const float* dL_drefl_strength_map, float* dL_dmean2D, float* dL_dnormal, float* dL_dopacity, float* dL_dcolor,
                                   float* dL_drefl_strengths, float* dL_dmean3D, float* dL_dtransMat, float* dL_dsh, float* dL_dscale,
                                   float* dL_drot, int accumulate, int debug, void* stream_) {
	return gsr_surfel_backward_ex(P, D, M, R, background, width, height, means3D, shs, colors_precomp, refl_strengths, scales, scale_modifier, rotations,
	                              transMat_precomp, viewmatrix, projmatrix, cam_pos, tan_fovx, tan_fovy, radii, geom_buffer, binning_buffer, image_buffer,
	                              dL_dpix, dL_dothers, dL_drefl_strength_map, dL_dmean2D, dL_dnormal, dL_dopacity, dL_dcolor, dL_drefl_strengths, dL_dmean3D,
	                              dL_dtransMat, dL_dsh, dL_dscale, dL_drot, accumulate, nullptr, debug, stream_);
}
```

Before: 549.8.

## Fold backward accumulator and cubemap scratch zeroing into forward kernels

Replaces the per-backward hipMemsetAsync of the per-Gaussian gradient accumulator with a nontemporal clear done by otherwise idle waves of the emit kernel, plus a device flag that lets a cheap fill kernel skip when the buffer is already clean. The reflection cubemap gradient scratch is now cleared by the forward preprocess kernel and re-zeroed by the unpack kernel after reading, so the backward memset is skipped when keys are pre-sorted. This removes two large memsets from the backward critical path, at the cost of extra stores inside forward kernels, an extra small kernel launch, and state-tracking flags that must stay consistent across calls.

Result: no change. 553.0, median of 6 (+0.6%).

```diff
diff --git a/gaussian-splatting-reflection_amd/csrc/gsr_common.hip b/gaussian-splatting-reflection_amd/csrc/gsr_common.hip
--- a/gaussian-splatting-reflection_amd/csrc/gsr_common.hip
+++ b/gaussian-splatting-reflection_amd/csrc/gsr_common.hip
@@ -56,9 +56,8 @@
 int option_cull() { return g_opt_cull; }
 static int g_opt_dev = 0;
 int option_dev() { return g_opt_dev; }
-unsigned long long* dev_pair_counter() {
+static unsigned long long* dev_counter(unsigned long long** words) {
 	static std::mutex mu;
-	static unsigned long long* words[64];
 	int dev = 0;
 	if (hipGetDevice(&dev) != hipSuccess || dev < 0 || dev >= 64) return nullptr;
 	std::lock_guard<std::mutex> lk(mu);
@@ -67,6 +66,14 @@
 		if (hipMemset(words[dev], 0, sizeof(unsigned long long)) != hipSuccess) return nullptr;
 	}
 	return words[dev];
+}
+unsigned long long* dev_pair_counter() {
+	static unsigned long long* words[64];
+	return dev_counter(words);
+}
+unsigned long long* dev_fill_counter() {
+	static unsigned long long* words[64];
+	return dev_counter(words);
 }
 static int g_opt_emit_items = 0;
 static int g_opt_mailbox = 1;
@@ -159,7 +166,8 @@
 	g.bbox = c.take<float4>(2 * P);
 	g.aux = c.take<float>(P * layout.aux_floats);
 	g.acc = c.take<float>(P * layout.acc_floats);
-	g.flags = c.take<int>(4);
+	g.acc_bytes = P * layout.acc_floats * sizeof(float);
+	g.flags = c.take<int>(8);
 	g.depth_sorted = c.take<uint32_t>(P);
 	g.order = c.take<unsigned long long>(P);
 	g.emit_state_bytes = ((((P + 255) / 256 + 1) * sizeof(unsigned long long)) + 15) & ~(size_t)15;
@@ -276,7 +284,8 @@
                                                          unsigned long long* __restrict__ scan_state, uint32_t* __restrict__ ticket,
                                                          uint32_t* __restrict__ tile_keys, uint32_t* __restrict__ vals, uint32_t tiles_x,
                                                          uint2* __restrict__ ranges, uint32_t tiles, void* sort_clear, size_t sort_clear_bytes,
-                                                         unsigned long long* __restrict__ blend_mask, size_t blend_words) {
+                                                         unsigned long long* __restrict__ blend_mask, size_t blend_words, void* acc_clear, size_t acc_clear_bytes,
+                                                         int* __restrict__ acc_clean) {
 	__shared__ uint32_t s_wsum[EMIT_BLOCK / 64];
 	__shared__ uint32_t s_base;
 	__shared__ uint32_t s_bid;
@@ -350,6 +359,10 @@
 			if (lane == 0u) emit_publish(scan_state + bid, emit_pack(2u, prefix + total));
 		}
 		if (lane == 0u) s_base = prefix;
+	} else {
+		const size_t cthreads = (size_t)gridDim.x * (EMIT_BLOCK - 64);
+		sort_clear_region_nt(acc_clear, acc_clear_bytes, (size_t)bid * (EMIT_BLOCK - 64) + (threadIdx.x - 64u), cthreads);
+		if (acc_clean != nullptr && bid == 0 && threadIdx.x == 64u) *acc_clean = 1;
 	}
 	__syncthreads();
 	uint32_t wbase = s_base;
@@ -563,11 +576,13 @@
 			const size_t clear_bytes = with_tile_sort((size_t)R, bit, [&](auto sort) { return sort.cleared_bytes((size_t)R, (unsigned)bit); });
 			uint32_t* ticket = reinterpret_cast<uint32_t*>(geom.emit_state + (geom.emit_state_bytes / sizeof(unsigned long long) - 1));
 			const int items = g_opt_emit_items ? g_opt_emit_items : (P >= EMIT_ITEMS2_FROM ? 2 : 1);
+			const bool acc_prepared = geom.acc_bytes != 0 && !(option_dev() & 16);
 			auto emit = rect_packs(tiles_x, tiles_y) ? (items == 2 ? emit_tiles_kernel<false, 2> : emit_tiles_kernel<false, 1>)
 			                                         : (items == 2 ? emit_tiles_kernel<true, 2> : emit_tiles_kernel<true, 1>);
 			emit<<<(P + EMIT_BLOCK * items - 1) / (EMIT_BLOCK * items), EMIT_BLOCK, 0, stream>>>(P, geom.order, geom.rect, geom.emit_state, ticket, b.tile_keys_unsorted,
 			                                                       b.vals_unsorted, (uint32_t)tiles_x, img.ranges, tiles, b.sort_temp, clear_bytes, b.blend_mask,
-			                                                       16 * b.mask_stride);
+			                                                       16 * b.mask_stride, acc_prepared ? geom.acc : nullptr, acc_prepared ? geom.acc_bytes : 0,
+			                                                       acc_prepared ? geom.flags + FLAG_ACC_CLEAN : nullptr);
 		}
 		GSR_LAUNCH_CHECK(debug, stream);
 		{
@@ -589,6 +604,25 @@
 		if (rc < 0) return rc;
 	}
 	return R;
+}
+
+#define ACC_FILL_BLOCKS 2048
+__global__ void __launch_bounds__(256) acc_fill_kernel(void* acc, size_t bytes, const int* __restrict__ clean, unsigned long long* __restrict__ fills) {
+	if (clean != nullptr && *clean == 1) return;
+	sort_clear_region(acc, bytes, (size_t)blockIdx.x * 256u + threadIdx.x, (size_t)gridDim.x * 256u);
+	if (fills != nullptr && blockIdx.x == 0 && threadIdx.x == 0) atomicAdd(fills, 1ull);
+}
+int ensure_acc_zero(const GeomState& geom, hipStream_t stream) {
+	unsigned long long* fills = nullptr;
+	if (option_dev() & 8) {
+		fills = dev_fill_counter();
+		if (!fills) { set_error("backward: no fill counter"); return GSR_E_HIP; }
+	}
+	if (geom.acc_bytes == 0 && !fills) return 0;
+	const unsigned blocks = (unsigned)std::min<size_t>(ACC_FILL_BLOCKS, std::max<size_t>(1, (geom.acc_bytes / 16 + 255) / 256));
+	acc_fill_kernel<<<blocks, 256, 0, stream>>>(geom.acc, geom.acc_bytes, geom.acc_bytes ? geom.flags + FLAG_ACC_CLEAN : nullptr, fills);
+	GSR_LAUNCH_CHECK(0, stream);
+	return 0;
 }
 
 int run_tile_order(const ImageState& img, size_t tiles, hipStream_t stream) {
@@ -708,6 +742,11 @@
 		if (!word) { set_error("gsr_debug_fetch: no pair counter"); return GSR_E_HIP; }
 		return d2d(word, sizeof(unsigned long long));
 	}
+	if (n == "fills") {
+		const unsigned long long* word = dev_fill_counter();
+		if (!word) { set_error("gsr_debug_fetch: no fill counter"); return GSR_E_HIP; }
+		return d2d(word, sizeof(unsigned long long));
+	}
 	if (n == "depths") return d2d(g.depths, (size_t)P * 4);
 	if (n == "means2D") return gather(0, 2);
 
diff --git a/gaussian-splatting-reflection_amd/csrc/gsr_cubemap.hip b/gaussian-splatting-reflection_amd/csrc/gsr_cubemap.hip
--- a/gaussian-splatting-reflection_amd/csrc/gsr_cubemap.hip
+++ b/gaussian-splatting-reflection_amd/csrc/gsr_cubemap.hip
@@ -345,18 +345,21 @@
 }
 
 template <bool ACC>
-__global__ void __launch_bounds__(256) unpack_cubemap_grad_kernel(const float4* __restrict__ scratch, float* __restrict__ g_cubemap,
+__global__ void __launch_bounds__(256) unpack_cubemap_grad_kernel(float4* __restrict__ scratch, float* __restrict__ g_cubemap,
                                                                   float* __restrict__ g_fail, int L) {
+	const float4 zero = make_float4(0.f, 0.f, 0.f, 0.f);
 	const size_t n = (size_t)6 * L * L;
 	const size_t t = (size_t)blockIdx.x * 256 + threadIdx.x;
 	if (t == 0) {
 		const float4 gf = scratch[n];
+		scratch[n] = zero;
 		g_fail[0] = (ACC ? g_fail[0] : 0.f) + gf.x; g_fail[1] = (ACC ? g_fail[1] : 0.f) + gf.y; g_fail[2] = (ACC ? g_fail[2] : 0.f) + gf.z;
 	}
 	if (t >= n) return;
 	const size_t LL = (size_t)L * L;
 	const size_t f = t / LL, r = t - f * LL;
 	const float4 g = scratch[t];
+	scratch[t] = zero;
 	float* o = g_cubemap + f * 3 * LL + r;
 	o[0] = (ACC ? o[0] : 0.f) + g.x;
 	o[LL] = (ACC ? o[LL] : 0.f) + g.y;
@@ -643,6 +646,18 @@
 	return 0;
 }
 
+int refl_zeroed_region(uint32_t L, int width, int height, float* scratch, size_t scratch_floats, void** region, size_t* bytes) {
+	ReflTail t(L, width, height, nullptr);
+	if (!t.carve(scratch, scratch_floats)) {
+		set_error("reflection backward (sorted footprints): scratch of %zu floats, 32-byte aligned, needed (gsr_deferred_reflection_scratch_floats(L, W, H, 1))",
+		          t.rs.total_floats);
+		return GSR_E_INVALID;
+	}
+	*region = t.staging;
+	*bytes = (size_t)(t.fail_acc + 4 - t.staging) * sizeof(float);
+	return 0;
+}
+
 int refl_sort_keys_early(uint32_t L, int width, int height, float* scratch, size_t scratch_floats, const uint32_t* sort_keys, int async, bool gated,
                          hipStream_t stream) {
 	ReflTail t(L, width, height, stream);
@@ -689,7 +704,7 @@
 	const bool binned = t.carve(scratch, scratch_floats);
 	if (keys_sorted && !binned) { set_error("gsr_deferred_reflection_backward: keys_sorted needs the scratch the forward sorted into"); return GSR_E_INVALID; }
 	auto unpack = accumulate ? unpack_cubemap_grad_kernel<true> : unpack_cubemap_grad_kernel<false>;
-	GSR_HIP_CHECK(hipMemsetAsync(scratch, 0, (ntex + 1) * 4 * sizeof(float), stream));
+	if (!keys_sorted || (option_dev() & 16)) GSR_HIP_CHECK(hipMemsetAsync(scratch, 0, (ntex + 1) * 4 * sizeof(float), stream));
 	if (!binned) {
 		{
 			StageTimer st_(GSR_STAGE_REFL_BWD, stream);
@@ -697,7 +712,7 @@
 			deferred_refl_bwd_kernel<<<grid, 256, 0, stream>>>(normal_view, base_color, refl_strength, cam, cubemap, fail_value, (int)L, width, height, g_final,
 			                                                  g_refl_color, g_normal_world, g_normal_view, g_base, g_strength, t.staging, t.fail_acc);
 		}
-		unpack<<<(unsigned)((ntex + 255) / 256), 256, 0, stream>>>((const float4*)t.staging, g_cubemap, g_fail, (int)L);
+		unpack<<<(unsigned)((ntex + 255) / 256), 256, 0, stream>>>((float4*)t.staging, g_cubemap, g_fail, (int)L);
 		GSR_LAUNCH_CHECK(0, stream);
 		return 0;
 	}
@@ -736,7 +751,7 @@
 		const unsigned cgrid = (unsigned)((t.rs.n + per_wg - 1) / per_wg);
 		if (!sort_keys) GSR_HIP_CHECK(t.sort(t.keys_in, small_sort, false));
 		refl_run_combine_kernel<<<cgrid, 256, 0, t.tail>>>(t.keys_out, t.pix_out, t.footprints, t.rs.n, L, (uint32_t)ntex, t.staging);
-		unpack<<<(unsigned)((ntex + 255) / 256), 256, 0, t.tail>>>((const float4*)t.staging, g_cubemap, g_fail, (int)L);
+		unpack<<<(unsigned)((ntex + 255) / 256), 256, 0, t.tail>>>((float4*)t.staging, g_cubemap, g_fail, (int)L);
 	}
 	if (t.side) GSR_HIP_CHECK(t.mark_done());
 	GSR_HIP_CHECK(hipGetLastError());
diff --git a/gaussian-splatting-reflection_amd/csrc/gsr_gauss.hip b/gaussian-splatting-reflection_amd/csrc/gsr_gauss.hip
--- a/gaussian-splatting-reflection_amd/csrc/gsr_gauss.hip
+++ b/gaussian-splatting-reflection_amd/csrc/gsr_gauss.hip
@@ -153,7 +153,7 @@
 	const int idx = blockIdx.x * 256 + threadIdx.x;
 	sort_clear_region(g.depth_sort_temp, g.depth_sort_clear, (size_t)idx, (size_t)gridDim.x * 256u);
 	sort_clear_region(g.emit_state, g.emit_state_bytes, (size_t)idx, (size_t)gridDim.x * 256u);
-	if (idx == 0) { g.flags[1] = 0; g.flags[2] = 0; g.flags[3] = 0; }
+	if (idx == 0) { g.flags[1] = 0; g.flags[2] = 0; g.flags[3] = 0; g.flags[FLAG_ACC_CLEAN] = 0; }
 	__shared__ float4 s_out[4][6 * 65];
 	const int lane = threadIdx.x & 63;
 	float4* so = s_out[threadIdx.x >> 6];
@@ -297,7 +297,8 @@
                              const float* __restrict__ final_Ts, const uint32_t* __restrict__ n_contrib, const float* __restrict__ dL_dpixels,
                              const float* __restrict__ dL_dnormal_map, const float* __restrict__ dL_drefl_map,
                              const float* __restrict__ dL_invdepths, float* __restrict__ acc, const unsigned long long* __restrict__ blend_mask,
-                             size_t mask_stride) {
+                             size_t mask_stride, int* __restrict__ acc_clean) {
+	if (blockIdx.x == 0 && threadIdx.x == 0) *acc_clean = 0;
 	const uint32_t slot = xcd_slot(blockIdx.x);
 	if (slot >= (uint32_t)ntiles * 4u) return;
 	const TileBlock blk = tile_block(tile_order, slot, tiles_x);
@@ -716,7 +717,7 @@
 			auto kern = dL_invdepths ? gauss_render_bwd_wave_kernel<true> : gauss_render_bwd_wave_kernel<false>;
 			kern<<<nunits, 64, 0, stream>>>(img.ranges, img.tile_order, bin.point_list, width, height, tiles_x, ntiles, background, geom.rec, geom.bbox, option_cull(),
 			                                img.final_T, img.n_contrib, dL_dpix, dL_dnormal_map, dL_drefl_strength_map, dL_invdepths, geom.acc, bin.blend_mask,
-			                                bin.mask_stride);
+			                                bin.mask_stride, geom.flags + FLAG_ACC_CLEAN);
 		}
 		GSR_LAUNCH_CHECK(debug, stream);
 	}
diff --git a/gaussian-splatting-reflection_amd/csrc/gsr_internal.hpp b/gaussian-splatting-reflection_amd/csrc/gsr_internal.hpp
--- a/gaussian-splatting-reflection_amd/csrc/gsr_internal.hpp
+++ b/gaussian-splatting-reflection_amd/csrc/gsr_internal.hpp
@@ -66,6 +66,7 @@
 	float4* bbox;
 	float* aux;
 	float* acc;
+	size_t acc_bytes;
 	int* flags;
 	uint32_t* depth_sorted;
 	unsigned long long* order;
@@ -97,6 +98,7 @@
 #define S_ACC_F 20
 #define G_REC_F4 4
 #define G_ACC_F 16
+#define FLAG_ACC_CLEAN 4
 struct WorkspaceLayout {
 	int rec_f4, aux_floats, acc_floats;
 	int planes_T, planes_n;
@@ -136,13 +138,15 @@
 	return c;
 }
 
+int ensure_acc_zero(const GeomState& geom, hipStream_t stream);
+int option_dev();
 struct BackwardWorkspace { GeomState geom; ImageState img; BinningState bin; int tiles_x, ntiles; };
 static inline int backward_prologue(const char* entry, const char* func, const WorkspaceLayout& layout, int P, int M, int R, int width, int height,
                                     bool missing_pointer, const float* shs, const float* dL_dsh, const float* dL_drot, const float* also_aligned,
                                     const char* also_what, void* geom_buffer, void* binning_buffer, void* image_buffer, hipStream_t stream,
                                     BackwardWorkspace* w) {
 	if (P < 0 || R < 0 || width <= 0 || height <= 0) { set_error("%s: invalid size", entry); return GSR_E_INVALID; }
-	if (P == 0) return 0;
+	if (P == 0) return (option_dev() & 8) && ensure_acc_zero(GeomState{}, stream) < 0 ? GSR_E_HIP : 0;
 	if (missing_pointer) { set_error("%s: missing required pointer", entry); return GSR_E_INVALID; }
 	if (shs && ((M * 3) & 3) == 0) GSR_REQUIRE_ALIGNED16_IN(func, shs, "shs (rows of a multiple of 16 bytes)");
 	if (shs && ((M * 3) & 3) == 0) GSR_REQUIRE_ALIGNED16_IN(func, dL_dsh, "dL_dsh");
@@ -153,13 +157,13 @@
 	w->geom = carve_geom(geom_buffer, P, layout, nullptr);
 	w->img = carve_image(image_buffer, (size_t)width * height, w->ntiles, layout, nullptr);
 	w->bin = carve_binning(binning_buffer, R, w->ntiles, 0, nullptr);
-	GSR_HIP_CHECK(hipMemsetAsync(w->geom.acc, 0, (size_t)P * layout.acc_floats * sizeof(float), stream));
-	return 1;
+	return ensure_acc_zero(w->geom, stream) < 0 ? GSR_E_HIP : 1;
 }
 
 int option_cull();
 int option_dev();
 unsigned long long* dev_pair_counter();
+unsigned long long* dev_fill_counter();
 size_t sort_temp_bytes(size_t R, int end_bit);
 int run_tile_order(const ImageState& img, size_t tiles, hipStream_t stream);
 uint32_t higher_msb(uint32_t n);
@@ -168,6 +172,7 @@
                 const ImageState& img, BinningState* out_binning, int prefiltered, int debug, hipStream_t stream, bool blend_masks = true);
 
 int side_gate_wait(hipStream_t stream);
+int refl_zeroed_region(uint32_t L, int width, int height, float* scratch, size_t scratch_floats, void** region, size_t* bytes);
 int refl_sort_keys_early(uint32_t L, int width, int height, float* scratch, size_t scratch_floats, const uint32_t* sort_keys, int async, bool gated,
                          hipStream_t stream);
 
diff --git a/gaussian-splatting-reflection_amd/csrc/gsr_sort.hpp b/gaussian-splatting-reflection_amd/csrc/gsr_sort.hpp
--- a/gaussian-splatting-reflection_amd/csrc/gsr_sort.hpp
+++ b/gaussian-splatting-reflection_amd/csrc/gsr_sort.hpp
@@ -139,6 +139,12 @@
 	uint4* p = static_cast<uint4*>(ptr);
 	for (size_t i = thread; i < bytes / 16; i += threads) p[i] = make_uint4(0u, 0u, 0u, 0u);
 }
+__device__ __forceinline__ void sort_clear_region_nt(void* ptr, size_t bytes, size_t thread, size_t threads) {
+	typedef uint32_t v4u __attribute__((ext_vector_type(4)));
+	v4u* p = static_cast<v4u*>(ptr);
+	const v4u zero = {0u, 0u, 0u, 0u};
+	for (size_t i = thread; i < bytes / 16; i += threads) __builtin_nontemporal_store(zero, p + i);
+}
 
 template <class T> const T* sort_values_in(T* p) { return p; }
 template <class It> It sort_values_in(It it) { return it; }
diff --git a/gaussian-splatting-reflection_amd/csrc/gsr_surfel.hip b/gaussian-splatting-reflection_amd/csrc/gsr_surfel.hip
--- a/gaussian-splatting-reflection_amd/csrc/gsr_surfel.hip
+++ b/gaussian-splatting-reflection_amd/csrc/gsr_surfel.hip
@@ -186,6 +186,8 @@
 	const float* cubemap;
 	float4* rgba;
 	uint32_t ntex, LL;
+	void* zero;
+	size_t zero_bytes;
 };
 template <bool TRAIN>
 __global__ void __launch_bounds__(256)
@@ -200,9 +202,10 @@
 		const float* c = ci.cubemap + (size_t)f * 3 * ci.LL + r;
 		ci.rgba[t] = make_float4(c[0], c[ci.LL], c[2 * (size_t)ci.LL], 0.f);
 	}
+	sort_clear_region(ci.zero, ci.zero_bytes, (size_t)idx, (size_t)gridDim.x * 256u);
 	sort_clear_region(g.depth_sort_temp, g.depth_sort_clear, (size_t)idx, (size_t)gridDim.x * 256u);
 	sort_clear_region(g.emit_state, g.emit_state_bytes, (size_t)idx, (size_t)gridDim.x * 256u);
-	if (idx == 0) { g.flags[1] = 0; g.flags[2] = 0; g.flags[3] = 0; }
+	if (idx == 0) { g.flags[1] = 0; g.flags[2] = 0; g.flags[3] = 0; g.flags[FLAG_ACC_CLEAN] = 0; }
 	__shared__ float4 s_out[4][S_REC_F4 * 65];
 	const int lane = threadIdx.x & 63;
 	float4* so = s_out[threadIdx.x >> 6];
@@ -817,7 +820,8 @@
                               const float* __restrict__ bg, const float4* __restrict__ rec, int dev_flags, const float* __restrict__ final_Ts,
                               const uint32_t* __restrict__ n_contrib, const float* __restrict__ dL_dpixels, const float* __restrict__ dL_depths,
                               const float* __restrict__ dL_drefl_map, const float* __restrict__ dL_dnormal_extra, float* __restrict__ acc,
-                              const unsigned long long* __restrict__ blend_mask) {
+                              const unsigned long long* __restrict__ blend_mask, int* __restrict__ acc_clean) {
+	if (blockIdx.x == 0 && threadIdx.x == 0) *acc_clean = 0;
 	surfel_render_bwd_rows_body(ranges, tile_order, point_list, W, H, tiles_x, ntiles, bg, rec, dev_flags, final_Ts, n_contrib, dL_dpixels, dL_depths,
 	                            dL_drefl_map, dL_dnormal_extra, acc, blend_mask);
 }
@@ -1039,6 +1043,12 @@
 	return refl_sort_keys_early(refl->L, width, height, refl->scratch, refl->scratch_floats, refl->sort_keys, refl->async_sort, R > 0, stream);
 }
 
+static int early_sort_zeroed_region(const gsr_refl_forward* refl, int width, int height, void** region, size_t* bytes) {
+	*region = nullptr; *bytes = 0;
+	if (!refl || !refl->sort_keys || !refl->scratch || (option_dev() & 16)) return 0;
+	return refl_zeroed_region(refl->L, width, height, refl->scratch, refl->scratch_floats, region, bytes);
+}
+
 template <bool TRAIN>
 static int surfel_forward(gsr_alloc_fn alloc, void* alloc_user, int P, int D, int M, const float* background, int width, int height,
                           const float* means3D, const uint8_t* env_scope_mask, const float* shs, const float* colors_precomp,
@@ -1049,6 +1059,9 @@
                           const gsr_refl_forward* refl, int debug, hipStream_t stream) {
 	const size_t HW = (size_t)width * height;
 	int R = 0;
+	void* refl_zero = nullptr;
+	size_t refl_zero_bytes = 0;
+	if (TRAIN) { if (const int rc = early_sort_zeroed_region(refl, width, height, &refl_zero, &refl_zero_bytes); rc < 0) return rc; }
 	if (P == 0) {
 		float* normal = TRAIN ? out_others + 2 * HW : out_normal_view;
 		if (!normal) {
@@ -1063,6 +1076,7 @@
 			GSR_HIP_CHECK(hipMemsetAsync(normal, 0, HW * 3 * 4, stream));
 		}
 		GSR_HIP_CHECK(hipMemsetAsync(out_refl_strength_map, 0, HW * 4, stream));
+		if (refl_zero_bytes) GSR_HIP_CHECK(hipMemsetAsync(refl_zero, 0, refl_zero_bytes, stream));
 		if (refl && gsr_deferred_reflection_forward_keys(normal, out_color, out_refl_strength_map, refl->cam, refl->cubemap, refl->fail_value, refl->L,
 		                                                 width, height, refl->out_final, refl->out_refl_color, refl->out_normal_world, refl->cubemap_rgba,
 		                                                 refl->sort_keys, stream) < 0)
@@ -1075,10 +1089,10 @@
 
 		if (prefiltered) GSR_HIP_CHECK(hipMemsetAsync(geom.flags, 0, 4 * sizeof(int), stream));
 		const RasterCam cam = make_cam(viewmatrix, projmatrix, cam_pos, width, height, tan_fovx, tan_fovy);
-		CubemapInterleave ci{nullptr, nullptr, 0u, 1u};
+		CubemapInterleave ci{nullptr, nullptr, 0u, 1u, nullptr, 0};
 		SurfelReflFwd rf{};
 		if (refl) {
-			ci = CubemapInterleave{refl->cubemap, reinterpret_cast<float4*>(refl->cubemap_rgba), 6u * refl->L * refl->L, refl->L * refl->L};
+			ci = CubemapInterleave{refl->cubemap, reinterpret_cast<float4*>(refl->cubemap_rgba), 6u * refl->L * refl->L, refl->L * refl->L, refl_zero, refl_zero_bytes};
 			rf = SurfelReflFwd{refl->cam, refl->cubemap, reinterpret_cast<const float4*>(refl->cubemap_rgba), refl->fail_value, (int)refl->L, 6u * refl->L * refl->L,
 			                   refl->out_final, refl->out_refl_color, refl->out_normal_world, refl->sort_keys};
 		}
@@ -1192,7 +1206,7 @@
 		const int nunits = (int)xcd_grid((uint32_t)ntiles * 4u);
 		surfel_render_bwd_rows_kernel<<<nunits, 64, 0, stream>>>(img.ranges, img.tile_order, bin.point_list, width, height, tiles_x, ntiles, background, geom.rec,
 		                                                         option_dev(), img.final_T, img.n_contrib, dL_dpix, dL_dothers, dL_drefl_strength_map, dL_dnormal_extra,
-		                                                         geom.acc, bin.blend_mask); }
+		                                                         geom.acc, bin.blend_mask, geom.flags + FLAG_ACC_CLEAN); }
 		GSR_LAUNCH_CHECK(debug, stream);
 	}
 	const RasterCam cam = make_cam(viewmatrix, projmatrix, cam_pos, width, height, tan_fovx, tan_fovy);
```
